# microsoft/UniSpeech

Measured on AMD Instinct MI355X. Metric: audio-seconds/sec pretraining, WavLM-Base 15s@16kHz, higher is better.
Workload: dtype bf16; 1 GPU; WavLM-Base (12L, d=768) pretrain fwd+bwd+grad-reduce+fused-Adam, bf16, batch=32x15s per GPU, masked-pred loss (BASELINE.json configs[1]); global_batch=32, frames_per_utt=749, parallelism=dp1, optimizer=fused Adam, fp32 master, clip 10

## Files before the change

### unispeech_amd/csrc/attn_fused.hip

```cpp
#include "attn_fused.hpp"

typedef float f32x2_t __attribute__((ext_vector_type(2)));
#if !defined(WAVLM_EXPERIMENTAL)
#undef FA_FWD_LAZY
#undef FA_FWD_THETA
#undef FA_DQ_PK
#endif
#ifndef FA_FWD_LAZY
#define FA_FWD_LAZY 0
#endif
#ifndef FA_FWD_THETA
#define FA_FWD_THETA 8.f
#endif
#ifndef FA_DQ_PK
#define FA_DQ_PK 1
#endif
#if !defined(WAVLM_EXPERIMENTAL)
#undef FA_FWD_MFMA_SUM
#endif
#ifndef FA_FWD_MFMA_SUM
#define FA_FWD_MFMA_SUM 0
#endif
#ifndef FA_FWD_BIAS_IN_C
#define FA_FWD_BIAS_IN_C 1
#endif
#ifndef FA_DQ_BIAS_IN_C
#define FA_DQ_BIAS_IN_C 0
#endif

template <bool DROP, bool STORE = false, bool BSTORE = false>
__global__ __launch_bounds__(256, 3) void attn_fwd_kernel(FaP p) {
  static_assert(!STORE || (FA_FWD_BIAS_IN_C && !FA_FWD_LAZY), "the probability store is written for the default forward");
  static_assert(!BSTORE || (DROP && !STORE && FA_FWD_BIAS_IN_C && !FA_FWD_LAZY), "the bit store is written for the default forward with dropout");
  extern __shared__ __attribute__((aligned(16))) unsigned char smem[];
  auto kbuf = [&](int st) { return smem + st * 16384; };
  auto vbuf = [&](int st) { return smem + st * 16384 + 8192; };
  float* tabs = reinterpret_cast<float*>(smem + 32768);
  float* kb = tabs + p.Ltab;
  unsigned* colw = reinterpret_cast<unsigned*>(kb + p.Tkb);
  const int T = p.T, H = p.H;
  int qblk, bh;
  fa_block_map(p.nqb, p.B * H, qblk, bh);
  const int b = bh / H, h = bh % H;
  const int lane = threadIdx.x & 63, wave = threadIdx.x >> 6;
  const int wave_u = __builtin_amdgcn_readfirstlane(wave);
  const int hi = lane >> 5, ql = lane & 31;
  const int i = qblk * FA_BQ + 32 * wave + ql;
  const int ic = i < T ? i : T - 1;
  const long D3 = 3L * H * FA_HD;
  const bf16_t* base = p.qkv + (long)b * T * D3 + h * FA_HD;
  const int L = 2 * T - 1;

  U4 qf[4];
#pragma unroll
  for (int kk = 0; kk < 4; ++kk) qf[kk].v = *reinterpret_cast<const uint4*>(base + (long)ic * D3 + 16 * kk + 8 * hi);
  for (int d = threadIdx.x; d < p.Ltab; d += 256) tabs[d] = (p.tab && d < L) ? p.tab[(long)h * L + d] : 0.f;
  for (int j = threadIdx.x; j < p.Tkb; j += 256)
    kb[j] = (j < T && !(p.kpm && p.kpm[(long)b * T + j])) ? 0.f : -INFINITY;
  if constexpr (DROP)
    for (int jp = threadIdx.x; jp < (p.Tkb >> 1); jp += 256) colw[jp] = fa_col_word(p.s1, (unsigned)jp);
  const float g2 = p.gate ? p.gate[(long)bh * T + ic] * FA_LOG2E : 0.f;
#if FA_FWD_BIAS_IN_C
  const float g2s = g2 / p.sc2;
#endif
  const unsigned roww = fa_row_word(p.s0, (unsigned)(bh * T + ic));
  const float* trow = tabs + (T - 1 - ic);

  f32x16_t o[2];
#pragma unroll
  for (int f = 0; f < 2; ++f)
#pragma unroll
    for (int r = 0; r < 16; ++r) o[f][r] = 0.f;
  float m = -INFINITY, l = 0.f;
#if FA_FWD_LAZY
  float mref = 0.f;
  bool seen = false;
#endif
  const int nkv = (T + FA_BKV - 1) / FA_BKV;
  const unsigned vtr = fa_tr_base(lane);
  unsigned* dbp = nullptr;
  if constexpr (BSTORE) dbp = p.dbits + ((long)bh * p.db_nkb + hi) * p.db_Tq + fa_bitrow(i);
  unsigned char* pst = nullptr;
  float* mtp = nullptr;
// ... 653 lines not shown
      }
    };
    auto dq_acc = [&](auto fc) __attribute__((always_inline)) {
      constexpr int f = decltype(fc)::value;
#pragma unroll
      for (int f2 = 0; f2 < 2; ++f2)
#pragma unroll
        for (int s2 = 0; s2 < 2; ++s2)
          dq[f2] = __builtin_amdgcn_mfma_f32_32x32x16_bf16(frag_tr(kbuf(cur), ktr, f2, f, s2), (f == 0 ? dsf0[s2] : dsf1[s2]).b, dq[f2], 0, 0, 0);
    };
#if FA_DQ_BOTH
    scores(F0{}); scores(F1{});
    if (edge) { elem_pass(F0{}, std::true_type{}); elem_pass(F1{}, std::true_type{}); }
    else { elem_pass(F0{}, std::false_type{}); elem_pass(F1{}, std::false_type{}); }
    dq_acc(F0{}); dq_acc(F1{});
#else
    scores(F0{});
    if (edge) elem_pass(F0{}, std::true_type{}); else elem_pass(F0{}, std::false_type{});
    dq_acc(F0{});
    scores(F1{});
    if (edge) elem_pass(F1{}, std::true_type{}); else elem_pass(F1{}, std::false_type{});
    dq_acc(F1{});
#endif
    if constexpr (EMIT) {
      auto spread = [&](unsigned a) __attribute__((always_inline)) {
        unsigned x = __builtin_bitreverse32(a) >> 16;
        x = (x | (x << 8)) & 0x00FF00FFu;
        x = (x | (x << 4)) & 0x0F0F0F0Fu;
        return x << (4 * hi);
      };
      unsigned w0 = spread(bacc0), w1 = spread(bacc1);
      asm volatile("s_nop 1\n\tv_permlane32_swap_b32 %0, %1\n\ts_nop 1" : "+v"(w0), "+v"(w1));
      pend_bits = w0 | w1;
      pend_bits_jt = jt;
      bacc0 = 0; bacc1 = 0;
    }
    if constexpr (TAB && !FA_DQ_DEFER) skew_sums(j0);
    fa_tile_sync<SP ? 5 : 0>();
    cur ^= 1;
  };
  if constexpr (SP) {
    for (int pi = 0; pi < (nkv >> 1); ++pi) {
      tile_body(2 * pi, pA0, pA1, mtA);
      tile_body(2 * pi + 1, pB0, pB1, mtB);
    }
    if (nkv & 1) tile_body(nkv - 1, pA0, pA1, mtA);
  } else {
    for (int jt = 0; jt < nkv; ++jt) tile_body(jt, pA0, pA1, mtA);
  }
  if constexpr (TAB && FA_DQ_DEFER) skew_sums((nkv - 1) * FA_BKV);
  if constexpr (TAB) flush_pending();
  if constexpr (EMIT)
    if (dbp && pend_bits_jt >= 0) dbp[(long)pend_bits_jt * 2 * p.db_Tq] = pend_bits;
  if (TAB && lane < 32) {
    const float v = lane < 16 ? dacc[4][0] : dacc[5][0];
    const int d = dlo0 + 64 * nkv + lane;
    if (d >= 0 && d < L) prow[d] = v;
  }
#if FA_DQ_PK
  dg = dg2[0] + dg2[1];
#endif
  dg = wl_sum_xor32(dg);
  if (p.dbias_part)
    fa_wave_colsum(dq, p.scale, reinterpret_cast<float*>(smem),
                   p.dbias_part + (((long)b * p.nqb + qblk) * 4 + wave_u) * D3 + h * FA_HD, lane, wave_u);
  if (valid_i) {
    bf16_t* dst = p.dqkv + ((long)b * T + i) * D3 + h * FA_HD;
#pragma unroll
    for (int f2 = 0; f2 < 2; ++f2)
#pragma unroll
      for (int q4 = 0; q4 < 4; ++q4) {
        uint2 w;
        w.x = pack_bf16(dq[f2][4 * q4] * p.scale, dq[f2][4 * q4 + 1] * p.scale);
        w.y = pack_bf16(dq[f2][4 * q4 + 2] * p.scale, dq[f2][4 * q4 + 3] * p.scale);
        *reinterpret_cast<uint2*>(dst + 32 * f2 + 8 * q4 + 4 * hi) = w;
      }
    if (hi == 0) {
      p.delta[(long)bh * T + i] = dl;
      if (p.dgate) p.dgate[(long)bh * T + i] = dg;
    }
  }
}

__global__ __launch_bounds__(1024) void fa_dtab_reduce_kernel(const float* __restrict__ part, float* __restrict__ out,
                                                              int B, int H, int nqt, int L, int Lp, int T, int nkv, int accumulate) {
  __shared__ float4 red[64][17];
  const int col = threadIdx.x & 15, slice = threadIdx.x >> 4;
  const int d = (blockIdx.x * 16 + col) * 4;
  const int h = blockIdx.y;
  const int nrow = nqt * 4, ntot = B * nrow, span = 64 * nkv + 32;
  float4 acc[4];
#pragma unroll
  for (int u = 0; u < 4; ++u) acc[u] = make_float4(0.f, 0.f, 0.f, 0.f);
  if (d < Lp) {
    for (int r0 = slice; r0 < ntot; r0 += 256) {
#pragma unroll
      for (int u = 0; u < 4; ++u) {
        const int r = r0 + 64 * u;
        if (r < ntot) {
          const int b = r / nrow, c = r - b * nrow;
          const int k0 = d - (T - 1 - 32 * c - 31);
          if (k0 > -4 && k0 < span) {
            const float4 v = *reinterpret_cast<const float4*>(part + (((long)b * H + h) * nrow + c) * Lp + d);
            acc[u].x += (k0 >= 0 && k0 < span) ? v.x : 0.f;
            acc[u].y += (k0 + 1 >= 0 && k0 + 1 < span) ? v.y : 0.f;
            acc[u].z += (k0 + 2 >= 0 && k0 + 2 < span) ? v.z : 0.f;
            acc[u].w += (k0 + 3 >= 0 && k0 + 3 < span) ? v.w : 0.f;
          }
        }
      }
    }
  }
  float4 t;
  t.x = (acc[0].x + acc[1].x) + (acc[2].x + acc[3].x); t.y = (acc[0].y + acc[1].y) + (acc[2].y + acc[3].y);
  t.z = (acc[0].z + acc[1].z) + (acc[2].z + acc[3].z); t.w = (acc[0].w + acc[1].w) + (acc[2].w + acc[3].w);
  red[slice][col] = t;
  __syncthreads();
  if (slice < 4) {
    float4 q = make_float4(0.f, 0.f, 0.f, 0.f);
#pragma unroll
    for (int k = 0; k < 16; ++k) { const float4 v = red[slice * 16 + k][col]; q.x += v.x; q.y += v.y; q.z += v.z; q.w += v.w; }
    red[slice * 16][col] = q;
  }
  __syncthreads();
  if (slice == 0 && d < L) {
    const float4 a0 = red[0][col], a1 = red[16][col], a2 = red[32][col], a3 = red[48][col];
    const float o[4] = {(a0.x + a1.x) + (a2.x + a3.x), (a0.y + a1.y) + (a2.y + a3.y), (a0.z + a1.z) + (a2.z + a3.z),
                        (a0.w + a1.w) + (a2.w + a3.w)};
#pragma unroll
    for (int k = 0; k < 4; ++k)
      if (d + k < L) out[(long)h * L + d + k] = accumulate ? out[(long)h * L + d + k] + o[k] : o[k];
  }
}

static FaP fa_params(int B, int H, int T, float scale, float p_drop, uint64_t seed) {
  FaP p;
  p.B = B; p.H = H; p.T = T; p.scale = scale;
  p.sc2 = scale * FA_LOG2E;
  double tt = (double)p_drop * 65536.0 + 0.5; if (tt > 65535.0) tt = 65535.0;
  p.th = p_drop > 0.f ? (unsigned)tt : 0u;
  if (p_drop > 0.f && p.th == 0u) p.th = 1u;
  p.sc = p.th ? (float)(1.0 / (1.0 - (double)p.th / 65536.0)) : 1.f;
  p.log2sc = log2f(p.sc); p.inv_sc = 1.f / p.sc;
  p.ths = (int)p.th - 32768;
  p.k2 = (unsigned)((p.ths - 1) & 0xffff) * 0x10001u;
  p.k3 = (unsigned)(p.ths & 0xffff) * 0x10001u;
  p.ps.P16 = nullptr; p.ps.mt = nullptr;
  p.dbits = nullptr; p.db_fwd = 0; p.db_nkb = ((T + FA_BKV - 1) / FA_BKV) * 2; p.db_Tq = ((T + FA_BQ - 1) / FA_BQ) * FA_BQ;
  p.ps.nq32 = ((T + FA_BQ - 1) / FA_BQ) * 4; p.ps.nkv = (T + FA_BKV - 1) / FA_BKV; p.ps.Tq = ((T + FA_BQ - 1) / FA_BQ) * FA_BQ;
  p.s0 = (unsigned)seed; p.s1 = (unsigned)(seed >> 32);
  const int nkv = (T + FA_BKV - 1) / FA_BKV;
  p.Tkb = nkv * FA_BKV;
  p.Ltab = (T + p.Tkb + 3) & ~3;
  p.qkv = nullptr; p.O = nullptr; p.lse = nullptr; p.gate = nullptr; p.tab = nullptr; p.kpm = nullptr;
  p.dO = nullptr; p.dqkv = nullptr; p.delta = nullptr; p.dgate = nullptr; p.dtab_part = nullptr; p.dbias_part = nullptr;
  return p;
}

extern "C" {

uint64_t wavlm_attn_fused_pstore_bytes(int32_t B, int32_t H, int32_t T) {
  if (B <= 0 || H <= 0 || T <= 0) return 0;
  if (T > FA_PSTORE_MAX_T) return 0;
  return ((fa_pstore_p_bytes(B, H, T) + 255) & ~(uint64_t)255) + fa_pstore_mt_bytes(B, H, T);
}

uint64_t wavlm_attn_fused_dbits_bytes(int32_t B, int32_t H, int32_t T) {
  if (B <= 0 || H <= 0 || T <= 0) return 0;
  return fa_dbits_bytes(B, H, T);
}

int wavlm_attn_fused_fwd(const void* qkv, void* O, float* lse, const float* gate, const float* tab, const uint8_t* kpm,
                         int32_t B, int32_t H, int32_t T, int32_t head_dim, float scale, float p_drop, uint64_t seed,
                         void* stream) {
  return wavlm_attn_fused_fwd_p(qkv, O, lse, gate, tab, kpm, nullptr, 0, B, H, T, head_dim, scale, p_drop, seed, stream);
}

static void fa_bind_pstore(FaP& p, void* pstore, int B, int H, int T) {
  p.ps.P16 = (unsigned char*)pstore;
  p.ps.mt = (float*)((unsigned char*)pstore + ((fa_pstore_p_bytes(B, H, T) + 255) & ~(uint64_t)255));
}

int wavlm_attn_fused_fwd_p(const void* qkv, void* O, float* lse, const float* gate, const float* tab, const uint8_t* kpm,
                           void* pstore, uint64_t pstore_bytes, int32_t B, int32_t H, int32_t T, int32_t head_dim, float scale,
                           float p_drop, uint64_t seed, void* stream) {
  if (!qkv || !O || !lse || B <= 0 || H <= 0 || T <= 0 || head_dim != FA_HD) return WL_EINVAL;
  if ((gate == nullptr) != (tab == nullptr)) return WL_EINVAL;
  const bool bitmode = pstore && pstore_bytes == fa_dbits_bytes(B, H, T);
  if (bitmode) { if ((uintptr_t)pstore & 255) return WL_EINVAL; }
  else if (pstore && (T > FA_PSTORE_MAX_T || pstore_bytes < wavlm_attn_fused_pstore_bytes(B, H, T) || ((uintptr_t)pstore & 15))) return WL_EINVAL;
  FaP p = fa_params(B, H, T, scale, p_drop, seed);
  p.qkv = (const bf16_t*)qkv; p.O = (bf16_t*)O; p.lse = lse; p.gate = gate; p.tab = tab; p.kpm = kpm;
  if (bitmode) { p.dbits = (unsigned*)pstore; p.db_fwd = 1; pstore = nullptr; }
  if (pstore) fa_bind_pstore(p, pstore, B, H, T);
  const size_t smem = 32768 + (size_t)(p.Ltab + p.Tkb + p.Tkb / 2) * sizeof(float);
  p.nqb = (T + FA_BQ - 1) / FA_BQ;
  const dim3 grid((unsigned)(p.nqb * B * H));
  WlProfScope prof(WL_PROF_ATTN_FWD, WL_BF16, 4.0 * B * H * (double)T * T * FA_HD,
                   (double)B * T * H * FA_HD * 2.0 * 4.0 + (double)B * H * T * 4.0, (hipStream_t)stream);
#define FA_FWD(DR, ST) do { if (fa_set_smem(attn_fwd_kernel<DR, ST>, smem) != WL_OK) return WL_ELAUNCH; \
    WL_LAUNCH((attn_fwd_kernel<DR, ST>), grid, dim3(256), smem, (hipStream_t)stream, p); } while (0)
  if (p.th && p.dbits) {
    if (fa_set_smem(attn_fwd_kernel<true, false, true>, smem) != WL_OK) return WL_ELAUNCH;
    WL_LAUNCH((attn_fwd_kernel<true, false, true>), grid, dim3(256), smem, (hipStream_t)stream, p);
  } else
  if (p.th) { if (pstore) FA_FWD(true, true); else FA_FWD(true, false); }
  else { if (pstore) FA_FWD(false, true); else FA_FWD(false, false); }
#undef FA_FWD
  return wl_check_launch();
}

uint64_t wavlm_attn_fused_bwd_workspace_bytes(int32_t B, int32_t H, int32_t T) {
  const uint64_t nqt = (uint64_t)((T + FA_BQ - 1) / FA_BQ);
  const uint64_t Lp = (2 * (uint64_t)T - 1 + 3) & ~(uint64_t)3;
  const uint64_t f = ((uint64_t)B * H * nqt * 4 * Lp + (uint64_t)B * H * T + (uint64_t)B * nqt * 4 * 3 * H * FA_HD) * sizeof(float);
// ... 22 lines not shown
}

int wl_attn_fused_bwd_ex(const void* qkv, const void* O, const void* dO, const float* lse, const float* gate,
                         const float* tab, const uint8_t* kpm, const void* pstore, uint64_t pstore_bytes, void* dqkv, float* dgate,
                         float* dtab, int dtab_accumulate,
                         void* dbias, int32_t dbias_dtype, int32_t dbias_accumulate, int32_t B, int32_t H, int32_t T,
                         int32_t head_dim, float scale, float p_drop, uint64_t seed, void* workspace, uint64_t ws_bytes,
                         void* stream) {
  if (!qkv || !O || !dO || !lse || !dqkv || !workspace || B <= 0 || H <= 0 || T <= 0 || head_dim != FA_HD)
    return WL_EINVAL;
  if ((gate == nullptr) != (tab == nullptr)) return WL_EINVAL;
  if (tab && (!dgate || !dtab)) return WL_EINVAL;
  if (ws_bytes < wavlm_attn_fused_bwd_workspace_bytes(B, H, T)) return WL_EINVAL;
  hipStream_t st = (hipStream_t)stream;
  FaP p = fa_params(B, H, T, scale, p_drop, seed);
  p.qkv = (const bf16_t*)qkv; p.O = (bf16_t*)const_cast<void*>(O); p.lse = const_cast<float*>(lse);
  p.gate = gate; p.tab = tab; p.kpm = kpm; p.dO = (const bf16_t*)dO; p.dqkv = (bf16_t*)dqkv; p.dgate = dgate;
  const unsigned* fwd_bits = nullptr;
  if (pstore && pstore_bytes == fa_dbits_bytes(B, H, T)) { fwd_bits = (const unsigned*)pstore; pstore = nullptr; }
  if (pstore) fa_bind_pstore(p, const_cast<void*>(pstore), B, H, T);
  const int nqt = (T + FA_BQ - 1) / FA_BQ;
  const int L = 2 * T - 1;
  p.dtab_part = (float*)workspace;
  const int Lp = (L + 3) & ~3;
  p.delta = p.dtab_part + (long)B * H * nqt * 4 * Lp;
  if (dbias) p.dbias_part = p.delta + (long)B * H * T;
  static const bool dbits_on = []() { const char* e = getenv("WAVLM_ATTN_DBITS"); return e && e[0] == '1'; }();
  static const bool dkv64_on = []() { const char* e = getenv("WAVLM_ATTN_DKV64"); return e && e[0] == '1'; }();
  bool use64 = dkv64_on && dbits_on && !pstore;
  if (use64) {
    FaP q = p; q.nqb = (T + FA_K64 - 1) / FA_K64;
    if (fa_dkv64_smem(q) > 160 * 1024) use64 = false;
  }
  if (fwd_bits && p.th) {
    p.dbits = const_cast<unsigned*>(fwd_bits); p.db_fwd = 1; use64 = false;
  } else
  if (dbits_on && !pstore && p.th) {
    const uint64_t fbytes = ((uint64_t)B * H * nqt * 4 * Lp + (uint64_t)B * H * T + (uint64_t)B * nqt * 4 * 3 * H * FA_HD) * sizeof(float);
    p.dbits = (unsigned*)((unsigned char*)workspace + ((fbytes + 255) & ~(uint64_t)255));
  }
  size_t smem1 = 32768 + (tab ? 4 * FA_SKEW_WAVE : 0) + (size_t)(p.Ltab + p.Tkb + p.Tkb / 2) * sizeof(float) + 256;
  if (smem1 < FA_CS_FLOATS * sizeof(float)) smem1 = FA_CS_FLOATS * sizeof(float);
  p.nqb = nqt;
  WlProfScope prof(WL_PROF_ATTN_BWD, WL_BF16, 10.0 * B * H * (double)T * T * FA_HD,
                   (double)B * T * H * FA_HD * 2.0 * 8.0 + (double)B * H * T * 8.0, st);
#define FA_DQ(DR, TB, SP_) do { if (fa_set_smem(attn_bwd_dq_kernel<DR, TB, SP_>, smem1) != WL_OK) return WL_ELAUNCH; \
    WL_LAUNCH((attn_bwd_dq_kernel<DR, TB, SP_>), dim3((unsigned)(nqt * B * H)), dim3(256), smem1, st, p); } while (0)
#define FA_DQB(TB) do { if (fa_set_smem(attn_bwd_dq_kernel<true, TB, false, true>, smem1) != WL_OK) return WL_ELAUNCH; \
    WL_LAUNCH((attn_bwd_dq_kernel<true, TB, false, true>), dim3((unsigned)(nqt * B * H)), dim3(256), smem1, st, p); } while (0)
  if (p.th && p.db_fwd) {
    if (tab) FA_DQB(true); else FA_DQB(false);
  } else
  if (pstore) {
    if (tab) FA_DQ(false, true, true); else FA_DQ(false, false, true);
  } else if (p.th && p.dbits) {
    if (tab) { if (fa_set_smem(attn_bwd_dq_kernel<true, true, false, false, true>, smem1) != WL_OK) return WL_ELAUNCH;
               WL_LAUNCH((attn_bwd_dq_kernel<true, true, false, false, true>), dim3((unsigned)(nqt * B * H)), dim3(256), smem1, st, p); }
    else { if (fa_set_smem(attn_bwd_dq_kernel<true, false, false, false, true>, smem1) != WL_OK) return WL_ELAUNCH;
           WL_LAUNCH((attn_bwd_dq_kernel<true, false, false, false, true>), dim3((unsigned)(nqt * B * H)), dim3(256), smem1, st, p); }
  } else if (p.th) {
    if (tab) FA_DQ(true, true, false); else FA_DQ(true, false, false);
  } else {
    if (tab) FA_DQ(false, true, false); else FA_DQ(false, false, false);
  }
#undef FA_DQ
#undef FA_DQB
  size_t smem2 = 32768 + (size_t)(p.Ltab + 64) * sizeof(float) + 2 * 4096;
  if (smem2 < FA_CS_FLOATS * sizeof(float)) smem2 = FA_CS_FLOATS * sizeof(float);
  if (use64) {
    p.nqb = (T + FA_K64 - 1) / FA_K64;
    const int rc = fa_launch_dkv64(p, (unsigned)(p.nqb * B * H), st);
    if (rc != WL_OK) return rc;
  } else {
    p.nqb = (T + FA_BK1 - 1) / FA_BK1;
    const dim3 grid2((unsigned)(p.nqb * B * H));
    const int rc = fa_launch_dkv(p, grid2.x, smem2, st);
    if (rc != WL_OK) return rc;
  }
  if (dbias) {
    const int rcb = wl_colsum_finish(p.dbias_part, B * nqt * 4, 3 * H * FA_HD, dbias, dbias_dtype, dbias_accumulate, st);
    if (rcb != WL_OK) return rcb;
    if (dbias_accumulate && !wl_fin_active()) wl_notify_grad(dbias, (uint64_t)3 * H * FA_HD * wl_esize(dbias_dtype), stream);
  }
  if (tab)
    WL_LAUNCH(fa_dtab_reduce_kernel, dim3((unsigned)((Lp / 4 + 15) / 16), (unsigned)H), dim3(1024), 0, st,
              (const float*)p.dtab_part, dtab, (int)B, (int)H, nqt, L, Lp, (int)T, (T + FA_BKV - 1) / FA_BKV, (int)dtab_accumulate);
  return wl_check_launch();
}
```

### unispeech_amd/csrc/common.hpp

```cpp
#pragma once
#include <hip/hip_runtime.h>
#include <stdint.h>
#include <stdio.h>
#include <mutex>

#define WL_MAX_DEVICES 64

#define WL_OK 0
#define WL_EINVAL (-1)
#define WL_ELAUNCH (-2)
#define WL_ENOMEM (-3)

enum { WL_F32 = 0, WL_BF16 = 1, WL_I16 = 2 };

typedef unsigned short bf16_t;

__device__ __forceinline__ float bf2f(bf16_t v) {
  return __uint_as_float(((unsigned)v) << 16);
}
__device__ __forceinline__ bf16_t f2bf(float f) {
  const __bf16 h = (__bf16)f;
  return __builtin_bit_cast(bf16_t, h);
}
__device__ __forceinline__ unsigned pack_bf16x2(float a, float b) {
// ... 89 lines not shown
}

__device__ __forceinline__ unsigned hash32(unsigned x) {
  x *= 0x9E3779B1u;
  x ^= x >> 15; x *= 0x85EBCA77u;
  x ^= x >> 13; x *= 0xC2B2AE3Du;
  x ^= x >> 16;
  return x;
}
__device__ __forceinline__ unsigned drop_mix(unsigned x) {
  x ^= x >> 16;
  unsigned r;
  asm("v_mul_u32_u24 %0, 0xb5297b, %1" : "=v"(r) : "v"(x));
  return r;
}
static inline unsigned drop_thresh16(float p) {
  if (p <= 0.f) return 0u;
  double t = (double)p * 65536.0 + 0.5;
  if (t > 65535.0) t = 65535.0;
  return t < 1.0 ? 1u : (unsigned)t;
}
static inline float drop_scale16(unsigned th16) { return th16 ? (float)(1.0 / (1.0 - (double)th16 / 65536.0)) : 1.f; }

struct Philox4 { unsigned x, y, z, w; };
__device__ __forceinline__ Philox4 philox4x32_10(unsigned long long seed, unsigned long long ctr) {
  unsigned k0 = (unsigned)seed, k1 = (unsigned)(seed >> 32);
  unsigned c0 = (unsigned)ctr, c1 = (unsigned)(ctr >> 32), c2 = 0x243F6A88u, c3 = 0x85A308D3u;
#pragma unroll
  for (int r = 0; r < 10; ++r) {
    const unsigned long long p0 = (unsigned long long)0xD2511F53u * c0;
    const unsigned long long p1 = (unsigned long long)0xCD9E8D57u * c2;
    const unsigned n0 = (unsigned)(p1 >> 32) ^ c1 ^ k0;
    const unsigned n1 = (unsigned)p1;
    const unsigned n2 = (unsigned)(p0 >> 32) ^ c3 ^ k1;
    const unsigned n3 = (unsigned)p0;
    c0 = n0; c1 = n1; c2 = n2; c3 = n3;
    k0 += 0x9E3779B9u; k1 += 0xBB67AE85u;
  }
  Philox4 o; o.x = c0; o.y = c1; o.z = c2; o.w = c3; return o;
}
__device__ __forceinline__ bool dropout_keep(unsigned long long seed, unsigned long long idx, unsigned thresh) {
  const Philox4 r = philox4x32_10(seed, idx >> 2);
  const unsigned sel = (unsigned)(idx & 3);
  const unsigned v = sel == 0 ? r.x : sel == 1 ? r.y : sel == 2 ? r.z : r.w;
  return v >= thresh;
}

static thread_local int wl_launch_failed = 0;
#define WL_LAUNCH(...)                                            \
  do {                                                            \
    (void)hipGetLastError();                                      \
    hipLaunchKernelGGL(__VA_ARGS__);                              \
    const hipError_t wl_e_ = hipGetLastError();                   \
    if (wl_e_ != hipSuccess) {                                    \
      wl_launch_failed = 1;                                       \
      fprintf(stderr, "[wavlm_hip] kernel launch failed: %s (%s:%d)\n", hipGetErrorString(wl_e_), __FILE__, __LINE__); \
    }                                                             \
  } while (0)
int wl_prof_begin(int cls, int dtype, double flops, double bytes, hipStream_t st);
void wl_prof_end(int i, hipStream_t st);
struct WlProfScope {
  int i; hipStream_t st;
  WlProfScope(int cls, int dtype, double flops, double bytes, hipStream_t s) : i(wl_prof_begin(cls, dtype, flops, bytes, s)), st(s) {}
  ~WlProfScope() { wl_prof_end(i, st); }
};

static inline int wl_check_launch() {
  const int e = wl_launch_failed;
  wl_launch_failed = 0;
  return e ? WL_ELAUNCH : WL_OK;
}

void wl_notify_grad(const void* base, uint64_t bytes, void* stream);
static inline uint64_t wl_esize(int dt) { return dt == WL_BF16 ? 2 : 4; }
int wl_attn_fused_bwd_ex(const void* qkv, const void* O, const void* dO, const float* lse, const float* gate,
                         const float* tab, const uint8_t* kpm, const void* pstore, uint64_t pstore_bytes, void* dqkv, float* dgate,
                         float* dtab, int dtab_accumulate,
                         void* dbias, int32_t dbias_dtype, int32_t dbias_accumulate, int32_t B, int32_t H, int32_t T,
                         int32_t head_dim, float scale, float p_drop, uint64_t seed, void* workspace, uint64_t ws_bytes,
                         void* stream);
int wl_colsum_finish(const float* part, int nblk, int n, void* out, int out_dtype, int accumulate, hipStream_t st);

struct WlFinSeg { const float* part; void* out; long stride, rep_stride; int nblk, n, out_dtype, accumulate, rep, blk0; };
#define WL_FIN_MAX 16
struct WlFinList { WlFinSeg s[WL_FIN_MAX]; int n, blocks; };
void wl_fin_defer(WlFinList* l);
bool wl_fin_active();
bool wl_fin_add(const float* part, int nblk, long stride, int n, void* out, int out_dtype, int accumulate, int rep = 1,
                long rep_stride = 0);
int wl_fin_flush(WlFinList& l, void* stream);
```

### unispeech_amd/csrc/gemm_bf16.hip

```cpp
#include <atomic>

#include "gemm_common.hpp"
#include "split_policy.hpp"

#include "tile_loaders.hpp"

template <bool TA, bool TB, int BM, int BN, int WM, int WN, bool VEC>
__global__ __launch_bounds__(WM * WN * 64) void gemm_bf16_kernel(GemmP p) {
  constexpr int FM = BM / WM / 32, FN = BN / WN / 32;
  constexpr int NT = WM * WN * 64;
  static_assert((WM * WN == 4 || WM * WN == 8) && FM >= 1 && FN >= 1, "4 or 8 waves");
  constexpr int A_BYTES = BM * 128, B_BYTES = BN * 128;
  extern __shared__ __attribute__((aligned(16))) unsigned char smem[];

  int tile;
  {
    const int nt = p.tiles_m * p.tiles_n, bid = blockIdx.x;
    const int q = nt >> 3, rem = nt & 7, xcd = bid & 7, idx = bid >> 3;
    tile = (xcd < rem ? xcd * (q + 1) : rem * (q + 1) + (xcd - rem) * q) + idx;
  }
  const int tn = tile % p.tiles_n, tm = tile / p.tiles_n;
  const int z = blockIdx.y, split = blockIdx.z;
  const int zo = z / p.batch_i, zi = z % p.batch_i;
  const int m0 = tm * BM, n0 = tn * BN;
// ... 83 lines not shown
      }
  } else {
    constexpr int WCOLS = BN / WN;
    constexpr int EP_LD = WCOLS + 4;
    constexpr int CH = WCOLS / 8;
    float* ep = reinterpret_cast<float*>(smem) + wave * (32 * EP_LD);
    const int zo2 = zo, zi2 = zi;
#pragma unroll
    for (int i = 0; i < FM; ++i) {
#pragma unroll
      for (int j = 0; j < FN; ++j)
#pragma unroll
        for (int r = 0; r < 16; ++r)
          ep[((r & 3) + 8 * (r >> 2) + 4 * (lane >> 5)) * EP_LD + j * 32 + (lane & 31)] = acc[i][j][r];
      __syncthreads();
#pragma unroll
      for (int q = 0; q < (32 * CH) / 64; ++q) {
        const int id = lane + 64 * q;
        const int rl = id / CH, ch = id % CH;
        const int mm = m0 + wm * (BM / WM) + i * 32 + rl;
        const int nn = n0 + wn * WCOLS + ch * 8;
        if (mm < p.M && nn < p.N) {
          const float4 lo = *reinterpret_cast<const float4*>(ep + rl * EP_LD + ch * 8);
          const float4 hi = *reinterpret_cast<const float4*>(ep + rl * EP_LD + ch * 8 + 4);
          float v[8] = {lo.x, lo.y, lo.z, lo.w, hi.x, hi.y, hi.z, hi.w};
          gemm_store8(p, zo2, zi2, z, split, mm, nn, v);
        }
      }
      __syncthreads();
    }
  }
}

__global__ __launch_bounds__(256) void gemm_splitk_reduce_kernel(GemmP p, int nbatch) {
  const long mn = (long)p.M * p.N;
  const long total = mn * nbatch;
  for (long i = (long)blockIdx.x * blockDim.x + threadIdx.x; i < total; i += (long)gridDim.x * blockDim.x) {
    const int z = (int)(i / mn);
    const long r = i - (long)z * mn;
    float s = 0.f;
    for (int k = 0; k < p.split_k; ++k) s += p.ws[((long)z * p.split_k + k) * mn + r];
    gemm_epi_final(p, z / p.batch_i, z % p.batch_i, (int)(r / p.N), (int)(r % p.N), s);
  }
}

__global__ __launch_bounds__(256) void gemm_splitk_reduce8_kernel(GemmP p, int nbatch) {
  const long mn = (long)p.M * p.N;
  const long total8 = (mn * nbatch) >> 3;
  const int S = p.split_k;
  GemmP q = p;
  q.split_k = 1;
  for (long i8 = (long)blockIdx.x * blockDim.x + threadIdx.x; i8 < total8; i8 += (long)gridDim.x * blockDim.x) {
    const long i = i8 << 3;
    const int z = (int)(i / mn);
    const long r = i - (long)z * mn;
    const float* src = p.ws + (long)z * S * mn + r;
    float v[8];
#pragma unroll
    for (int e = 0; e < 8; ++e) v[e] = 0.f;
    int k = 0;
    for (; k + 4 <= S; k += 4) {
      float4 a[4], b[4];
#pragma unroll
      for (int u = 0; u < 4; ++u) {
        a[u] = *reinterpret_cast<const float4*>(src + (long)(k + u) * mn);
        b[u] = *reinterpret_cast<const float4*>(src + (long)(k + u) * mn + 4);
      }
#pragma unroll
      for (int u = 0; u < 4; ++u) {
        v[0] += a[u].x; v[1] += a[u].y; v[2] += a[u].z; v[3] += a[u].w;
        v[4] += b[u].x; v[5] += b[u].y; v[6] += b[u].z; v[7] += b[u].w;
      }
    }
    for (; k < S; ++k) {
      const float4 a = *reinterpret_cast<const float4*>(src + (long)k * mn);
      const float4 b = *reinterpret_cast<const float4*>(src + (long)k * mn + 4);
      v[0] += a.x; v[1] += a.y; v[2] += a.z; v[3] += a.w; v[4] += b.x; v[5] += b.y; v[6] += b.z; v[7] += b.w;
    }
    const int m = (int)(r / p.N), n = (int)(r - (long)m * p.N);
    gemm_store8(q, z / p.batch_i, z % p.batch_i, z, 0, m, n, v);
  }
}

struct RedGrpP {
  float* ws[4]; void* C[4]; long ldc[4]; int M[4], N[4], c_dtype[4], accumulate[4]; float alpha[4];
  long base[5]; int n, S;
};
__global__ __launch_bounds__(256) void gemm_splitk_reduce8_grouped_kernel(RedGrpP p) {
  const long total8 = p.base[p.n];
  for (long i8 = (long)blockIdx.x * blockDim.x + threadIdx.x; i8 < total8; i8 += (long)gridDim.x * blockDim.x) {
    const int g = (i8 >= p.base[1]) + (i8 >= p.base[2]) + (i8 >= p.base[3]);
    const long i = (i8 - p.base[g]) << 3;
    const int N = p.N[g];
    const long mn = (long)p.M[g] * N;
    const float* src = p.ws[g] + i;
    float v[8];
#pragma unroll
    for (int e = 0; e < 8; ++e) v[e] = 0.f;
    for (int k = 0; k < p.S; ++k) {
      const float4 a = *reinterpret_cast<const float4*>(src + (long)k * mn);
      const float4 b = *reinterpret_cast<const float4*>(src + (long)k * mn + 4);
      v[0] += a.x; v[1] += a.y; v[2] += a.z; v[3] += a.w; v[4] += b.x; v[5] += b.y; v[6] += b.z; v[7] += b.w;
    }
    const long m = i / N, n = i - m * N;
    const long off = m * p.ldc[g] + n;
#pragma unroll
    for (int e = 0; e < 8; ++e) v[e] *= p.alpha[g];
    if (p.accumulate[g]) {
      float c[8];
      ld8_dt(p.C[g], off, p.c_dtype[g], c);
#pragma unroll
      for (int e = 0; e < 8; ++e) v[e] += c[e];
    }
    st8_dt(p.C[g], off, p.c_dtype[g], v);
  }
}

template <bool TA, bool TB, int BM, int BN, int WM, int WN>
static int launch_cfg(GemmP& p, int nbatch, bool vec, hipStream_t st) {
  p.tiles_m = (p.M + BM - 1) / BM;
  p.tiles_n = (p.N + BN - 1) / BN;
  dim3 grid((unsigned)(p.tiles_m * p.tiles_n), (unsigned)nbatch, (unsigned)p.split_k);
  constexpr size_t smem = 2 * (size_t)(BM + BN) * 128;
  constexpr int nt = WM * WN * 64;
  if (smem > 65536) {
    static bool done_v = false, done_s = false;
    bool& done = vec ? done_v : done_s;
    if (!done) {
      const void* fn = vec ? (const void*)gemm_bf16_kernel<TA, TB, BM, BN, WM, WN, true>
                           : (const void*)gemm_bf16_kernel<TA, TB, BM, BN, WM, WN, false>;
      if (hipFuncSetAttribute(fn, hipFuncAttributeMaxDynamicSharedMemorySize, (int)smem) != hipSuccess) return WL_ELAUNCH;
      done = true;
    }
  }
  if (vec) WL_LAUNCH((gemm_bf16_kernel<TA, TB, BM, BN, WM, WN, true>), grid, dim3(nt), smem, st, p);
  else WL_LAUNCH((gemm_bf16_kernel<TA, TB, BM, BN, WM, WN, false>), grid, dim3(nt), smem, st, p);
  return wl_check_launch();
}

static int g_gemm_variant = 0;
extern int g_pp_mode;
extern "C" void wavlm_gemm_set_variant(int v) { g_gemm_variant = v & 15; if (v >> 4) g_pp_mode = (v >> 4) - 1; }

template <bool TA, bool TB>
static int launch_t(GemmP& p, int nbatch, bool vec, hipStream_t st) {
  if (p.N <= 64) return launch_cfg<TA, TB, 128, 64, 2, 2>(p, nbatch, vec, st);
  if (g_gemm_variant == 2 ||
      (g_gemm_variant == 0 && p.M >= 2048 && (long)((p.M + 255) / 256) * ((p.N + 127) / 128) * nbatch * p.split_k >= 192))
    return launch_cfg<TA, TB, 256, 128, 4, 2>(p, nbatch, vec, st);
  return launch_cfg<TA, TB, 128, 128, 2, 2>(p, nbatch, vec, st);
}

static bool vec_epilogue_ok(const wavlm_gemm_desc* d, bool final_stage = false) {
  auto ok = [](const void* ptr, int64_t a, int64_t b, int64_t c) {
    return (((uintptr_t)ptr) & 15) == 0 && a % 8 == 0 && b % 8 == 0 && c % 8 == 0;
  };
  if (d->split_k > 1 && !final_stage) return (((uintptr_t)d->workspace) & 15) == 0 && d->N % 8 == 0;
  if (final_stage && d->N % 8) return false;
  if (!ok(d->C, d->ldc, d->sC_o, d->sC_i)) return false;
  if (d->bias && !ok(d->bias, 0, d->sBias_o, d->sBias_i)) return false;
  if (d->aux && !ok(d->aux, d->ld_aux, d->sAux_o, d->sAux_i)) return false;
  if (d->res && !ok(d->res, d->ld_res, d->sRes_o, d->sRes_i)) return false;
  return true;
}

int gemm_f32_launch(const wavlm_gemm_desc* d, hipStream_t st);
bool gemm_pp_ok(const wavlm_gemm_desc* d);
int gemm_pp_launch(GemmP& p, int nbatch, bool transA, bool transB, int ep, hipStream_t st);
bool gemm_pp3_ok(const wavlm_gemm_desc* d);
int gemm_pp3_launch(GemmP& p, int nbatch, bool transA, bool transB, int ep, hipStream_t st);
#if defined(WAVLM_EXPERIMENTAL)
#define GEMM_LAB 1
bool gemm_h2_ok(const wavlm_gemm_desc* d, int ec);
int gemm_h2_launch(GemmP& p, bool transB, int ep, hipStream_t st);
static int h2_mode() { static const int m = getenv("WAVLM_GEMM_H2") ? atoi(getenv("WAVLM_GEMM_H2")) : -1; return m; }
static bool h2_takes(const wavlm_gemm_desc* d, int ec) {
  const int m = h2_mode();
  if (m == 0 || !gemm_h2_ok(d, ec)) return false;
  if (m == 1) return true;
  return false;
}
#else
#define GEMM_LAB 0
#endif
int gemm_w4_launch(GemmP& p, int nbatch, bool transA, bool transB, int ep, hipStream_t st);
int gemm_w4_launch_grouped(GemmP& p, hipStream_t st);
static int w4_mode() { static const int m = getenv("WAVLM_GEMM_W4") ? atoi(getenv("WAVLM_GEMM_W4")) : 3; return m; }
static bool w4_takes(const wavlm_gemm_desc* d, bool grouped) {
  const int m = w4_mode();
  if (m == 1) return true;
  if (m == 2) return grouped || (d->transA && d->transB);
  if (m == 3) return grouped;
  return false;
}

static double tile_efficiency(const wavlm_gemm_desc* d, int nbatch, int BM, int BN) {
  const long tm = (d->M + BM - 1) / BM, tn = (d->N + BN - 1) / BN;
  const long tiles = tm * tn * nbatch * (d->split_k < 1 ? 1 : d->split_k);
// ... 219 lines not shown
      long blocks = ((total >> 3) + 255) / 256; if (blocks > 2048) blocks = 2048;
      WL_LAUNCH(gemm_splitk_reduce8_kernel, dim3((unsigned)blocks), dim3(256), 0, st, p, nbatch);
    } else {
      long blocks = (total + 255) / 256; if (blocks > 4096) blocks = 4096;
      WL_LAUNCH(gemm_splitk_reduce_kernel, dim3((unsigned)blocks), dim3(256), 0, st, p, nbatch);
    }
    rc = wl_check_launch();
  }
  if (rc == WL_OK && d->colsum) {
    if (csum_rows > 0) rc = wl_colsum_finish((const float*)d->workspace, csum_rows, d->N, d->colsum, d->colsum_dtype, d->colsum_accumulate, st);
    else rc = wavlm_colsum(d->C, d->M, d->N, d->ldc, d->c_dtype, nullptr, nullptr, d->colsum, d->colsum_dtype,
                           d->colsum_accumulate, d->workspace, d->ws_bytes, stream);
  }
  prof_end(pi, st);
  if (rc == WL_OK) gemm_notify(d, csum_rows > 0, stream);
  return rc;
}

int gemm_pp_launch_grouped(GemmP& p, hipStream_t st);
bool gemm_w4_fixup_ok(const GemmP& p);

extern "C" int wavlm_gemm_grouped(const wavlm_gemm_desc* d, int32_t n, void* stream) {
  if (!d || n <= 0) return WL_EINVAL;
  hipStream_t st = (hipStream_t)stream;
  bool ok = n >= 2 && n <= 4;
  for (int i = 0; ok && i < n; ++i) {
    const wavlm_gemm_desc* e = d + i;
    ok = e->A && e->B && e->C && e->workspace && e->dtype == WL_BF16 && e->transA && e->transB && e->KB <= 1 &&
         e->batch_o <= 1 && e->batch_i <= 1 && e->K == d->K && e->split_k == d->split_k && e->split_k >= 2 &&
         e->epi == 0 && !e->bias && !e->aux && !e->res && e->M > 0 && e->N > 0 && gemm_pp_ok(e) &&
         aligned16(e->A) && aligned16(e->B) && e->lda % 8 == 0 && e->ldb % 8 == 0 &&
         vec_epilogue_ok(e) && vec_epilogue_ok(e, true) && e->ws_bytes >= wavlm_gemm_workspace_bytes(e);
  }
  if (!ok || g_gemm_variant != 0) {
    for (int i = 0; i < n; ++i) {
      const int rc = wavlm_gemm(d + i, stream);
      if (rc != WL_OK) return rc;
    }
    return WL_OK;
  }
  GemmP p = make_gemm_params(d);
  p.ngrp = n;
  long tiles_all = 0;
  for (int i = 0; i < n; ++i) tiles_all += (long)((d[i].M + 255) / 256) * ((d[i].N + 255) / 256);
  const int G = wl_policy::grid_blocks();
  const bool sk_on = wl_policy::streamk();
  const int ksteps = (d->K + 63) / 64;
  GemmSk plan;
  const bool sk = sk_on && w4_takes(d, true) && tiles_all * (long)ksteps >= 8l * G && gemm_sk_plan(tiles_all, ksteps, G, plan) &&
                  d->split_k >= plan.s + 1;
  if (sk) p.split_k = plan.s + 1;
  else if (sk_on && !wl_policy::forced_split() && G / tiles_all >= 2 && d->split_k == G / tiles_all + 1)
    p.split_k = (int)(G / tiles_all);
  int vb = 0;
  double flops = 0.0;
  for (int i = 0; i < 4; ++i) {
    const wavlm_gemm_desc* e = d + (i < n ? i : n - 1);
    GemmGrp& g = p.grp[i];
    g.A = e->A; g.B = e->B; g.ws = (float*)e->workspace; g.lda = e->lda; g.ldb = e->ldb; g.M = e->M; g.N = e->N;
    g.tiles_m = (e->M + 255) / 256; g.tiles_n = (e->N + 255) / 256;
    g.C = e->C; g.ldc = e->ldc; g.c_dtype = e->c_dtype; g.accumulate = e->accumulate; g.alpha = e->alpha;
    g.vbase = i < n ? vb : 0x7fffffff;
    if (i < n) { vb += g.tiles_m * g.tiles_n * (sk ? 1 : p.split_k); flops += 2.0 * e->M * e->N * (double)e->K; }
  }
  p.vtotal = vb;
  if (sk) {
    p.sk_ks = ksteps; p.sk_wgs = G; p.sk_tiles = (int)tiles_all; p.sk_s = plan.s; p.sk_lm = plan.Lm;
    p.vtotal = G * plan.q;
    static const bool spread = [] { const char* e = getenv("WAVLM_SK_SPREAD"); return !(e && *e == '0'); }();
    p.sk_spread = spread && (plan.s * tiles_all) % 8 == 0 && plan.R % 8 == 0 && G % 8 == 0;
  }
  const int pi = prof_begin(d, st);
  if (pi >= 0) {
    g_prof.flops[pi] = flops;
    double by = 0.0;
    for (int i = 0; i < n; ++i) by += 2.0 * ((double)d[i].M * d[i].K + (double)d[i].N * d[i].K) + 2.0 * 2.0 * d[i].M * d[i].N;
    g_prof.bytes[pi] = by;
    int* sh = g_prof.shape[pi];
    sh[0] = -n; sh[1] = 0; sh[2] = d->K; sh[3] = 1; sh[4] = 3; sh[5] = 0; sh[6] = sk ? 0 : p.split_k; sh[7] = n;
  }
  const bool fixup = w4_takes(d, true) && gemm_w4_fixup_ok(p);
  p.fix_epoch = fixup ? 1u : 0u; p.fix_cnt = nullptr; p.fix_flag = nullptr;
  int rc = w4_takes(d, true) ? gemm_w4_launch_grouped(p, st) : gemm_pp_launch_grouped(p, st);
  if (rc == WL_OK && !fixup) {
    RedGrpP r;
    r.n = n; r.S = p.split_k; r.base[0] = 0;
    for (int i = 0; i < 4; ++i) {
      const wavlm_gemm_desc* e = d + (i < n ? i : n - 1);
      r.ws[i] = (float*)e->workspace; r.C[i] = e->C; r.ldc[i] = e->ldc; r.M[i] = e->M; r.N[i] = e->N;
      r.c_dtype[i] = e->c_dtype; r.accumulate[i] = e->accumulate; r.alpha[i] = e->alpha;
      r.base[i + 1] = i < n ? r.base[i] + (((long)e->M * e->N) >> 3) : 0x7fffffffffffffffL;
    }
    const long total8 = r.base[n];
    long blocks = (total8 + 255) / 256; if (blocks > 4096) blocks = 4096;
    WL_LAUNCH(gemm_splitk_reduce8_grouped_kernel, dim3((unsigned)blocks), dim3(256), 0, st, r);
    rc = wl_check_launch();
  }
  prof_end(pi, st);
  if (rc == WL_OK)
    for (int i = 0; i < n; ++i) gemm_notify(d + i, false, stream);
  return rc;
}
```

### unispeech_amd/csrc/gemm_common.hpp

```cpp
#pragma once
#include <stdlib.h>
#include "common.hpp"
#include "../../include/wavlm_hip.h"

struct GemmGrp { const void* A; const void* B; float* ws; long lda, ldb; int M, N, tiles_m, tiles_n, vbase;
                 void* C; long ldc; int c_dtype, accumulate; float alpha; };

struct GemmP {
  const void* A; const void* B; void* C;
  int M, N, K, KB;
  long lda, ldb, ldc, sA_kb, sB_kb;
  int batch_i;
  long sA_o, sA_i, sB_o, sB_i, sC_o, sC_i;
  float alpha; int epi; int c_dtype;
  const void* bias; int bias_dtype; long sBias_o, sBias_i;
  void* aux; int aux_dtype; long ld_aux, sAux_o, sAux_i;
  const void* res; int res_dtype; long ld_res, sRes_o, sRes_i;
  int accumulate;
  int split_k; float* ws;
  int tiles_m, tiles_n;
  int vtotal, nbatch, skew;
  int swz_r;
  int patch_m;
  int ngrp;
  unsigned fix_epoch; unsigned* fix_cnt; unsigned* fix_flag;
  int sk_ks, sk_wgs, sk_tiles, sk_s, sk_lm, sk_spread;
  const float4* gtab;
  float* colsum_part;
  GemmGrp grp[4];
};

#define GEMM_SK_SEG_COST 8
struct GemmSk { int s, R, q, Lm; };
static inline bool gemm_sk_plan(long T, long KS, int G, GemmSk& k) {
  if (T <= 0 || T >= G) return false;
  k.s = (int)(G / T); k.R = (int)(G - T * k.s);
  if (k.R == 0 || k.s < 1) return false;
  k.q = (int)((T + k.R - 1) / k.R);
  static const long c_env = [] { const char* e = getenv("WAVLM_SK_SEG_COST"); return e && *e ? atol(e) : 0l; }();
  const long c = c_env > 0 ? c_env : GEMM_SK_SEG_COST;
  const long L0 = (k.q * (KS + c) - c) / (1 + (long)k.s * k.q);
  long Lm = 0, best = 0;
  for (long L = L0; L <= L0 + 1; ++L) {
    if (L < 8 || KS - L * k.s < 1) continue;
    const long tail = k.q * (KS - L * k.s + c), cost = L + c > tail ? L + c : tail;
    if (Lm == 0 || cost < best) { Lm = L; best = cost; }
  }
  if (Lm == 0 || best * 100 > 97 * ((KS + k.s - 1) / k.s + c)) return false;
  k.Lm = (int)Lm;
  return true;
}

__host__ __device__ inline void gemm_tile_rc(int tile, int tiles_m, int tiles_n, int R, int& tm, int& tn) {
  if (R <= 1) { tm = tile / tiles_n; tn = tile - tm * tiles_n; return; }
  const int per = R * tiles_n;
  const int sr = tile / per;
  int rows = tiles_m - sr * R; if (rows > R) rows = R;
  const int w = tile - sr * per;
  tn = w / rows; tm = sr * R + (w - tn * rows);
}
static inline int gemm_pick_swizzle(int tile_m, int tile_n, int tiles_m, int tiles_n, long b_bytes) {
  static const int off = getenv("WAVLM_GEMM_SWIZZLE") && getenv("WAVLM_GEMM_SWIZZLE")[0] == '0';
  if (off || tiles_n <= 1 || tiles_m <= 1 || b_bytes < 6l * 1000 * 1000) return 0;
  long best = -1; int br = 0;
  for (int R = 1; R <= 32; R *= 2) {
    if (R > tiles_m) break;
    int cols = (32 + R - 1) / R; if (cols > tiles_n) cols = tiles_n;
    int rows = R; if (cols * R < 32) { rows = (32 + cols - 1) / cols; if (rows > tiles_m) rows = tiles_m; }
    const long cost = (long)tile_m * rows + (long)tile_n * cols;
    if (best < 0 || cost < best) { best = cost; br = R; }
  }
  return br <= 1 ? 0 : br;
}

static inline GemmP make_gemm_params(const wavlm_gemm_desc* d) {
  GemmP p;
  p.A = d->A; p.B = d->B; p.C = d->C;
  p.M = d->M; p.N = d->N; p.K = d->K; p.KB = d->KB < 1 ? 1 : d->KB;
  p.lda = d->lda; p.ldb = d->ldb; p.ldc = d->ldc; p.sA_kb = d->sA_kb; p.sB_kb = d->sB_kb;
  p.batch_i = d->batch_i < 1 ? 1 : d->batch_i;
  p.sA_o = d->sA_o; p.sA_i = d->sA_i; p.sB_o = d->sB_o; p.sB_i = d->sB_i; p.sC_o = d->sC_o; p.sC_i = d->sC_i;
  p.alpha = d->alpha; p.epi = d->epi; p.c_dtype = d->c_dtype;
  p.bias = d->bias; p.bias_dtype = d->bias_dtype; p.sBias_o = d->sBias_o; p.sBias_i = d->sBias_i;
  p.aux = d->aux; p.aux_dtype = d->aux_dtype; p.ld_aux = d->ld_aux; p.sAux_o = d->sAux_o; p.sAux_i = d->sAux_i;
  p.gtab = nullptr;
  p.colsum_part = nullptr;
  p.res = d->res; p.res_dtype = d->res_dtype; p.ld_res = d->ld_res; p.sRes_o = d->sRes_o; p.sRes_i = d->sRes_i;
  p.accumulate = d->accumulate;
  p.split_k = d->split_k < 1 ? 1 : d->split_k;
  p.ws = (float*)d->workspace;
  p.tiles_m = 0; p.tiles_n = 0; p.vtotal = 0; p.nbatch = 1; p.skew = 0; p.patch_m = 0; p.ngrp = 0;
  p.sk_ks = 0; p.sk_wgs = 0; p.sk_tiles = 0; p.sk_s = 0; p.sk_lm = 0; p.sk_spread = 0;
  p.swz_r = 0;
  p.fix_epoch = 0; p.fix_cnt = nullptr; p.fix_flag = nullptr;
  return p;
}

__device__ __forceinline__ void gemm_epi_final(const GemmP& p, int zo, int zi, int m, int n, float acc) {
  float v = p.alpha * acc;
  if (p.bias) v += ld_elem(p.bias, (long)zo * p.sBias_o + (long)zi * p.sBias_i + n, p.bias_dtype);
  if (p.epi == 1) {
    if (p.aux) st_elem(p.aux, (long)zo * p.sAux_o + (long)zi * p.sAux_i + (long)m * p.ld_aux + n, p.aux_dtype, v);
    v = gelu_f(v);
  } else if (p.epi == 2) {
    const float u = ld_elem(p.aux, (long)zo * p.sAux_o + (long)zi * p.sAux_i + (long)m * p.ld_aux + n, p.aux_dtype);
    v *= gelu_grad_f(u);
  } else if (p.epi == 3) {
    float gr;
    v = gelu_both_f(v, gr);
    if (p.aux) st_elem(p.aux, (long)zo * p.sAux_o + (long)zi * p.sAux_i + (long)m * p.ld_aux + n, p.aux_dtype, gr);
  } else if (p.epi == 4) {
    v *= ld_elem(p.aux, (long)zo * p.sAux_o + (long)zi * p.sAux_i + (long)m * p.ld_aux + n, p.aux_dtype);
  }
  if (p.res) v += ld_elem(p.res, (long)zo * p.sRes_o + (long)zi * p.sRes_i + (long)m * p.ld_res + n, p.res_dtype);
  const long ci = (long)zo * p.sC_o + (long)zi * p.sC_i + (long)m * p.ldc + n;
  if (p.accumulate) v += ld_elem(p.C, ci, p.c_dtype);
  st_elem(p.C, ci, p.c_dtype, v);
}

__device__ __forceinline__ void gemm_store(const GemmP& p, int z, int split, int m, int n, float acc) {
  if (p.split_k > 1) {
    p.ws[((long)z * p.split_k + split) * ((long)p.M * p.N) + (long)m * p.N + n] = acc;
  } else {
    gemm_epi_final(p, z / p.batch_i, z % p.batch_i, m, n, acc);
  }
}


__device__ __forceinline__ void ld8_dt(const void* p, long idx, int dt, float (&v)[8]) {
  if (dt == WL_F32) {
    const float4 a = *reinterpret_cast<const float4*>((const float*)p + idx);
    const float4 b = *reinterpret_cast<const float4*>((const float*)p + idx + 4);
    v[0] = a.x; v[1] = a.y; v[2] = a.z; v[3] = a.w; v[4] = b.x; v[5] = b.y; v[6] = b.z; v[7] = b.w;
  } else {
    const uint4 a = *reinterpret_cast<const uint4*>((const bf16_t*)p + idx);
    v[0] = __uint_as_float(a.x << 16); v[1] = __uint_as_float(a.x & 0xffff0000u);
    v[2] = __uint_as_float(a.y << 16); v[3] = __uint_as_float(a.y & 0xffff0000u);
    v[4] = __uint_as_float(a.z << 16); v[5] = __uint_as_float(a.z & 0xffff0000u);
    v[6] = __uint_as_float(a.w << 16); v[7] = __uint_as_float(a.w & 0xffff0000u);
  }
}
__device__ __forceinline__ void st8_dt(void* p, long idx, int dt, const float (&v)[8]) {
  if (dt == WL_F32) {
    *reinterpret_cast<float4*>((float*)p + idx) = make_float4(v[0], v[1], v[2], v[3]);
    *reinterpret_cast<float4*>((float*)p + idx + 4) = make_float4(v[4], v[5], v[6], v[7]);
  } else {
    uint4 o;
    o.x = pack_bf16x2(v[0], v[1]); o.y = pack_bf16x2(v[2], v[3]);
    o.z = pack_bf16x2(v[4], v[5]); o.w = pack_bf16x2(v[6], v[7]);
    *reinterpret_cast<uint4*>((bf16_t*)p + idx) = o;
  }
}

__device__ __forceinline__ void gemm_store8(const GemmP& p, int zo, int zi, int z, int split, int m, int n,
                                            float (&acc)[8]) {
  if (n + 8 > p.N) {
    for (int e = 0; e < 8 && n + e < p.N; ++e) gemm_store(p, z, split, m, n + e, acc[e]);
    return;
  }
  if (p.split_k > 1) {
    float* dst = p.ws + ((long)z * p.split_k + split) * ((long)p.M * p.N) + (long)m * p.N + n;
    *reinterpret_cast<float4*>(dst) = make_float4(acc[0], acc[1], acc[2], acc[3]);
    *reinterpret_cast<float4*>(dst + 4) = make_float4(acc[4], acc[5], acc[6], acc[7]);
    return;
  }
  float v[8];
#pragma unroll
  for (int e = 0; e < 8; ++e) v[e] = p.alpha * acc[e];
  if (p.bias) {
    float b[8];
    ld8_dt(p.bias, (long)zo * p.sBias_o + (long)zi * p.sBias_i + n, p.bias_dtype, b);
#pragma unroll
    for (int e = 0; e < 8; ++e) v[e] += b[e];
  }
  if (p.epi == 1) {
    if (p.aux) st8_dt(p.aux, (long)zo * p.sAux_o + (long)zi * p.sAux_i + (long)m * p.ld_aux + n, p.aux_dtype, v);
#pragma unroll
    for (int e = 0; e < 8; ++e) v[e] = gelu_f(v[e]);
  } else if (p.epi == 2) {
    float u[8];
    ld8_dt(p.aux, (long)zo * p.sAux_o + (long)zi * p.sAux_i + (long)m * p.ld_aux + n, p.aux_dtype, u);
#pragma unroll
    for (int e = 0; e < 8; ++e) v[e] *= gelu_grad_f(u[e]);
  } else if (p.epi == 3) {
    float gr[8];
#pragma unroll
    for (int e = 0; e < 8; ++e) v[e] = gelu_both_f(v[e], gr[e]);
    if (p.aux) st8_dt(p.aux, (long)zo * p.sAux_o + (long)zi * p.sAux_i + (long)m * p.ld_aux + n, p.aux_dtype, gr);
  } else if (p.epi == 4) {
    float u[8];
    ld8_dt(p.aux, (long)zo * p.sAux_o + (long)zi * p.sAux_i + (long)m * p.ld_aux + n, p.aux_dtype, u);
#pragma unroll
    for (int e = 0; e < 8; ++e) v[e] *= u[e];
  }
  if (p.res) {
    float r[8];
    ld8_dt(p.res, (long)zo * p.sRes_o + (long)zi * p.sRes_i + (long)m * p.ld_res + n, p.res_dtype, r);
#pragma unroll
    for (int e = 0; e < 8; ++e) v[e] += r[e];
  }
  const long ci = (long)zo * p.sC_o + (long)zi * p.sC_i + (long)m * p.ldc + n;
  if (p.accumulate) {
    float c[8];
    ld8_dt(p.C, ci, p.c_dtype, c);
#pragma unroll
    for (int e = 0; e < 8; ++e) v[e] += c[e];
  }
  st8_dt(p.C, ci, p.c_dtype, v);
}

#define GT4_N 2048
#define GT2_N (2 * GT4_N)
__device__ __forceinline__ float gelu_both_tab(const float4* tab4, float x, float& grad) {
  const float2* tab = reinterpret_cast<const float2*>(tab4);
  float u = fmaf(x, GT2_N / 16.0f, 8.0f * (GT2_N / 16.0f));
  u = __builtin_amdgcn_fmed3f(u, 0.f, (float)(GT2_N - 1));
  const float2 t = tab[(int)u];
  const float ph = fmaf(t.x, x, t.y);
  grad = fmaf(x, t.x, ph);
  return x * ph;
}
const float4* wl_gelu_tab4(hipStream_t st);
__device__ __forceinline__ void gelu_tab_stage(const float4* g, float4* lds) {
  for (int i = threadIdx.x; i < GT4_N; i += blockDim.x) lds[i] = g[i];
}

__device__ __forceinline__ void gemm_unpack8(const uint4& a, float (&u)[8]) {
  u[0] = __uint_as_float(a.x << 16); u[1] = __uint_as_float(a.x & 0xffff0000u);
  u[2] = __uint_as_float(a.y << 16); u[3] = __uint_as_float(a.y & 0xffff0000u);
  u[4] = __uint_as_float(a.z << 16); u[5] = __uint_as_float(a.z & 0xffff0000u);
  u[6] = __uint_as_float(a.w << 16); u[7] = __uint_as_float(a.w & 0xffff0000u);
}
template <int KIND>
__device__ __forceinline__ void gemm_store8_fast(const GemmP& p, int zo, int zi, int m, int n, const float (&acc)[8],
                                                 const float4* tab = nullptr, float* vout = nullptr, const uint4* aux_pre = nullptr,
// ... 94 lines not shown
```

### unispeech_amd/csrc/layer.hip

```cpp
#include <stdlib.h>
#include <string.h>

#include <atomic>

#include "common.hpp"
#include "split_policy.hpp"
#include "wavlm_hip.h"

static std::atomic<wavlm_grad_listener> g_listener{nullptr};
static std::atomic<void*> g_listener_user{nullptr};
void wl_notify_grad(const void* base, uint64_t bytes, void* stream) {
  const wavlm_grad_listener cb = g_listener.load(std::memory_order_acquire);
  if (cb && base && bytes) cb(base, bytes, stream, g_listener_user.load(std::memory_order_acquire));
}
extern "C" void wavlm_dp_set_listener(wavlm_grad_listener cb, void* user) {
  g_listener.store(nullptr, std::memory_order_release);
  g_listener_user.store(user, std::memory_order_release);
  g_listener.store(cb, std::memory_order_release);
}

namespace {

inline uint64_t rup256(uint64_t v) { return (v + 255) & ~(uint64_t)255; }

// ... 91 lines not shown
  gemm_base(g);
  g.c_dtype = pdt; g.M = w.N; g.N = w.K; g.K = (int32_t)n; g.transA = 1; g.transB = 1;
  g.lda = w.N; g.ldb = w.K; g.ldc = w.K; g.A = w.dy; g.B = w.x; g.C = w.dW; g.accumulate = 1; g.split_k = split;
}
inline long wg_tiles(const wavlm_wgrad_item& w) { return (long)((w.N + 255) / 256) * ((w.K + 255) / 256); }

#define RC(expr) do { const int rc_ = (expr); if (rc_ != WL_OK) return rc_; } while (0)

struct BwdWs {
  void *dsa, *df, *du, *dh, *dxa, *da, *dO, *dqkv;
  float* dgate;
  void *ln_ws, *ln_ws2, *cs_ws, *cs_ws2, *attn_ws, *gate_ws, *wg_ws;
  uint64_t ln_b, cs_b, attn_b, gate_b, wg_b, bytes;
};
BwdWs carve_bwd(const wavlm_layer_desc* d, void* base, uint64_t cap) {
  BwdWs w; memset(&w, 0, sizeof(w));
  Carver c(base ? base : (void*)256, base ? cap : (~(uint64_t)0 >> 1));
  const uint64_t n = (uint64_t)d->B * d->T, D = d->D, F = d->F;
  w.dsa = c.take(n * D * 2);
  w.df = d->p_drop > 0.f ? c.take(n * D * 2) : w.dsa;
  w.du = c.take(n * F * 2);
  w.dh = c.take(n * D * 2);
  w.dxa = c.take(n * D * 2);
  w.da = d->p_drop > 0.f ? c.take(n * D * 2) : w.dxa;
  w.dO = c.take(n * D * 2);
  w.dqkv = c.take(n * 3 * D * 2);
  if (d->tab) w.dgate = (float*)c.take((uint64_t)d->B * d->H * d->T * 4);
  w.ln_b = wavlm_layernorm_bwd_workspace_bytes(d->D); w.ln_ws = c.take(w.ln_b); w.ln_ws2 = c.take(w.ln_b);
  w.cs_b = lin_dx_colsum_ws((int64_t)n, d->F);
  if (w.cs_b < wavlm_colsum_workspace_bytes(d->D)) w.cs_b = wavlm_colsum_workspace_bytes(d->D);
  w.cs_ws = c.take(w.cs_b); w.cs_ws2 = c.take(w.cs_b);
  w.attn_b = wavlm_attn_fused_bwd_workspace_bytes(d->B, d->H, d->T); w.attn_ws = c.take(w.attn_b);
  w.gate_b = wavlm_gate_bwd_workspace_bytes(d->H, 64); w.gate_ws = c.take(w.gate_b);
  const wavlm_wgrad_item it[4] = {{nullptr, nullptr, nullptr, d->D, d->F}, {nullptr, nullptr, nullptr, d->F, d->D},
                                  {nullptr, nullptr, nullptr, d->D, d->D}, {nullptr, nullptr, nullptr, 3 * d->D, d->D}};
  w.wg_b = wavlm_linear_wgrads_workspace_bytes(it, 4, (int64_t)n); w.wg_ws = c.take(w.wg_b);
  w.bytes = c.off;
  if (base && !c.ok) w.bytes = ~(uint64_t)0;
  return w;
}

}

#if defined(WAVLM_EXPERIMENTAL)
extern "C" int wavlm_lab_build(void) { return 1; }
#endif

extern "C" {

static long grid_or(int32_t grid) { return grid > 0 ? grid : wl_policy::grid_blocks(); }
static int forced_or(int32_t forced) { return forced >= 0 ? forced : wl_policy::forced_split(); }
int32_t wavlm_grid_blocks(void) { return wl_policy::grid_blocks(); }
int32_t wavlm_wgrad_grouping(void) { return wl_policy::grouping() ? 1 : 0; }
int32_t wavlm_split_single(int32_t M, int32_t N, int64_t ktiles, int32_t grid) { return wl_policy::split_single(M, N, (long)ktiles, grid_or(grid)); }
int32_t wavlm_split_grouped(int64_t tiles, int64_t ktiles, int32_t grid, int32_t forced) {
  return wl_policy::split_grouped((long)tiles, (long)ktiles, grid_or(grid), forced_or(forced));
}
int32_t wavlm_slabs_grouped(int64_t tiles, int64_t ktiles, int32_t grid, int32_t forced, int32_t balanced) {
  return wl_policy::slabs_grouped((long)tiles, (long)ktiles, grid_or(grid), forced_or(forced), balanced >= 0 ? balanced != 0 : wl_policy::streamk());
}

uint64_t wavlm_linear_wgrads_workspace_bytes(const wavlm_wgrad_item* it, int32_t cnt, int64_t n) {
  if (!it || cnt <= 0 || n <= 0) return 0;
  uint64_t tot = 0;
  const long kt = (long)((n + 63) / 64), G = wl_policy::kFullGrid;
  const int forced = wl_policy::forced_split();
  const bool balanced = wl_policy::streamk() && forced == 0;
  for (int i = 0; i < cnt; ++i) {
    const long t = wg_tiles(it[i]);
    int s = wl_policy::split_single(it[i].N, it[i].K, kt, G);
    const int gs = wl_policy::slabs_grouped(t, kt, G, forced, false);
    if (gs > s) s = gs;
    if (balanced && t < G && G / t + 1 > s) s = (int)(G / t) + 1;
    tot += rup256((uint64_t)s * it[i].N * it[i].K * 4);
  }
  return tot;
}

int wavlm_linear_wgrads(const wavlm_wgrad_item* it, int32_t cnt, int64_t n, int32_t pdt, void* ws, uint64_t wsb, void* stream) {
  if (!it || cnt <= 0 || n <= 0 || (pdt != WL_BF16 && pdt != WL_F32)) return WL_EINVAL;
  for (int i = 0; i < cnt; ++i)
    if (!it[i].dy || !it[i].x || !it[i].dW || it[i].N <= 0 || it[i].K <= 0) return WL_EINVAL;
  const long kt = (long)((n + 63) / 64);
  int i = 0;
  while (i < cnt) {
    int j = i; long tiles = 0;
    while (wl_policy::grouping() && j < cnt && j - i < 4) {
      const long t = wg_tiles(it[j]);
      if (j > i && wavlm_split_grouped(tiles + t, kt, 0, -1) < 2) break;
      tiles += t; ++j;
    }
    if (j == i) j = i + 1;
    const int m = j - i;
    Carver c(ws, wsb);
    if (m >= 2) {
      const int split = wavlm_slabs_grouped(tiles, kt, 0, -1, -1);
      wavlm_gemm_desc g[4];
      for (int k = 0; k < m; ++k) {
        wg_desc(g[k], it[i + k], n, pdt, split);
        g[k].ws_bytes = wavlm_gemm_workspace_bytes(&g[k]);
        g[k].workspace = c.take(g[k].ws_bytes);
      }
      if (!c.ok) return WL_EINVAL;
      const int rc = wavlm_gemm_grouped(g, m, stream);
      if (rc != WL_OK) return rc;
    } else {
      wavlm_gemm_desc g;
      wg_desc(g, it[i], n, pdt, wavlm_split_single(it[i].N, it[i].K, kt, 0));
      if (g.split_k > 1) { g.ws_bytes = wavlm_gemm_workspace_bytes(&g); g.workspace = c.take(g.ws_bytes); if (!c.ok) return WL_EINVAL; }
      const int rc = wavlm_gemm(&g, stream);
      if (rc != WL_OK) return rc;
    }
    i = j;
  }
  return WL_OK;
}

uint64_t wavlm_layer_saved_bytes(const wavlm_layer_desc* d) { return desc_ok(d) ? carve_saved(d, nullptr).bytes : 0; }

uint64_t wavlm_layer_fwd_workspace_bytes(const wavlm_layer_desc* d) {
  if (!desc_ok(d)) return 0;
  return rup256((uint64_t)d->B * d->T * d->D * 2) + (d->saved ? 0 : carve_saved(d, nullptr).bytes);
}

uint64_t wavlm_layer_bwd_workspace_bytes(const wavlm_layer_desc* d) { return desc_ok(d) ? carve_bwd(d, nullptr, 0).bytes : 0; }

int wavlm_encoder_layer_fwd(const wavlm_layer_desc* d, void* stream) {
  if (!desc_ok(d) || !d->x || !d->y || !d->workspace) return WL_EINVAL;
  if (d->pre_ln && !d->r_out) return WL_EINVAL;
  if (d->ws_bytes < wavlm_layer_fwd_workspace_bytes(d)) return WL_EINVAL;
  const int64_t n = (int64_t)d->B * d->T;
  const int D = d->D, F = d->F, pdt = d->param_dtype;
  Carver wc(d->workspace, d->ws_bytes);
  void* tmp = wc.take((uint64_t)n * D * 2);
  void* sbase = d->saved;
  if (sbase) { if (d->saved_bytes < carve_saved(d, nullptr).bytes) return WL_EINVAL; }
  else sbase = wc.take(carve_saved(d, nullptr).bytes);
  if (!wc.ok) return WL_EINVAL;
  const Saved s = carve_saved(d, sbase);

  const void* ain = d->x;
  if (d->pre_ln) {
    RC(wavlm_layernorm_fwd(d->x, d->r_in, s.h1, d->r_in ? s.s1 : nullptr, s.mean1, s.rstd1, d->ln1_g, d->ln1_b, n, D, d->eps1,
                           WL_BF16, pdt, 0, d->r_in ? d->p_drop : 0.f, d->seed_r1, 0.f, 0, stream));
    ain = s.h1;
  }
  const float* gate = nullptr;
  if (d->Wgate) {
    RC(wavlm_gate_fwd(ain, d->Wgate, d->bgate, d->grep_a, s.gate, s.ga, s.gb, d->B, d->T, d->H, 64, WL_BF16, pdt, stream));
    gate = s.gate;
  } else if (d->tab) {
    return WL_EINVAL;
  }
  RC(lin_fwd(ain, d->Wqkv, d->bqkv, s.qkv, n, 3 * D, D, pdt, 0, nullptr, stream));
  RC(wavlm_attn_fused_fwd_p(s.qkv, s.O, s.lse, gate, d->tab, d->kpm, d->saved ? s.pstore : nullptr, s.pstore_b, d->B, d->H, d->T, 64,
                            d->scale, d->p_attn, d->seed_attn, stream));
  RC(lin_fwd(s.O, d->Wo, d->bo, tmp, n, D, D, pdt, 0, nullptr, stream));
  if (!d->pre_ln) {
    RC(wavlm_layernorm_fwd(d->x, tmp, s.x1, s.s1, s.mean1, s.rstd1, d->ln1_g, d->ln1_b, n, D, d->eps1, WL_BF16, pdt, 0,
                           d->p_drop, d->seed_r1, 0.f, 0, stream));
    RC(lin_fwd(s.x1, d->W1, d->b1, s.hact, n, F, D, pdt, 3, s.u, stream));
    RC(lin_fwd(s.hact, d->W2, d->b2, tmp, n, D, F, pdt, 0, nullptr, stream));
    RC(wavlm_layernorm_fwd(s.x1, tmp, d->y, s.s2, s.mean2, s.rstd2, d->ln2_g, d->ln2_b, n, D, d->eps2, WL_BF16, pdt, 0,
                           d->p_drop, d->seed_r2, 0.f, 0, stream));
  } else {
    const void* s1 = d->r_in ? s.s1 : d->x;
    RC(wavlm_layernorm_fwd(s1, tmp, s.x1, d->y, s.mean2, s.rstd2, d->ln2_g, d->ln2_b, n, D, d->eps2, WL_BF16, pdt, 0,
                           d->p_drop, d->seed_r2, 0.f, 0, stream));
    RC(lin_fwd(s.x1, d->W1, d->b1, s.hact, n, F, D, pdt, 3, s.u, stream));
    RC(lin_fwd(s.hact, d->W2, d->b2, d->r_out, n, D, F, pdt, 0, nullptr, stream));
  }
  return WL_OK;
}

int wavlm_encoder_layer_bwd(const wavlm_layer_desc* d, void* stream) {
  if (!desc_ok(d) || !d->x || !d->dy || !d->dx || !d->saved || !d->workspace) return WL_EINVAL;
  if (!d->dWqkv || !d->dbqkv || !d->dWo || !d->dbo || !d->dW1 || !d->db1 || !d->dW2 || (!d->db2 && !d->pre_ln)) return WL_EINVAL;
// ... 71 lines not shown
```

### unispeech_amd/csrc/posconv.hip

```cpp
#include "common.hpp"
#include "../../include/wavlm_hip.h"

#define PC_BLOCKS 512

template <typename TA, typename TB>
__global__ void pc_rowdot_partial_kernel(const TA* __restrict__ a, const TB* __restrict__ b, long rows, int K,
                                         float* __restrict__ part) {
  const int k = threadIdx.x;
  if (k >= K) return;
  float s0 = 0.f, s1 = 0.f, s2 = 0.f, s3 = 0.f;
  const long G = gridDim.x;
  long r = blockIdx.x;
  for (; r + 3 * G < rows; r += 4 * G) {
    s0 = fmaf(Elem<TA>::ld(a + r * K + k), Elem<TB>::ld(b + r * K + k), s0);
    s1 = fmaf(Elem<TA>::ld(a + (r + G) * K + k), Elem<TB>::ld(b + (r + G) * K + k), s1);
    s2 = fmaf(Elem<TA>::ld(a + (r + 2 * G) * K + k), Elem<TB>::ld(b + (r + 2 * G) * K + k), s2);
    s3 = fmaf(Elem<TA>::ld(a + (r + 3 * G) * K + k), Elem<TB>::ld(b + (r + 3 * G) * K + k), s3);
  }
  for (; r < rows; r += G) s0 = fmaf(Elem<TA>::ld(a + r * K + k), Elem<TB>::ld(b + r * K + k), s0);
  part[(long)blockIdx.x * K + k] = (s0 + s1) + (s2 + s3);
}

__global__ __launch_bounds__(1024) void pc_finish_kernel(const float* __restrict__ part, int nblk, int K, float* __restrict__ tot, int do_sqrt) {
  __shared__ double red[64][17];
  const int col = threadIdx.x & 15, slice = threadIdx.x >> 4;
  const int k = blockIdx.x * 16 + col;
  double s = 0.0;
  if (k < K)
    for (int b = slice; b < nblk; b += 64) s += part[(long)b * K + k];
  red[slice][col] = s;
  __syncthreads();
  if (slice == 0 && k < K) {
    s = 0.0;
    for (int j = 0; j < 64; ++j) s += red[j][col];
    tot[k] = do_sqrt ? (float)sqrt(s) : (float)s;
  }
}

template <typename TP, typename TO>
__global__ __launch_bounds__(256) void pc_weight_kernel(const TP* __restrict__ v, const TP* __restrict__ g,
    const float* __restrict__ norm, TO* __restrict__ Wf, TO* __restrict__ Wb, int D, int Cg, int K, int layout) {
  const long total = (long)D * Cg * K;
  const long KC = (long)K * Cg;
  auto off = [&](int grp, int n, int tap, int c) -> long {
    if (layout == 0) return ((long)grp * Cg + n) * KC + (long)tap * Cg + c;
    const int J = K >> 4;
    return (long)grp * Cg * KC + (((((long)(c >> 3) * 4 + ((tap & 15) >> 2)) * J + (tap >> 4)) * 4 + (tap & 3)) * Cg + n) * 8 + (c & 7);
  };
  for (long i = (long)blockIdx.x * blockDim.x + threadIdx.x; i < total; i += (long)gridDim.x * blockDim.x) {
    const int k = (int)(i % K);
    const long r = i / K;
    const int ci = (int)(r % Cg), co = (int)(r / Cg);
    const int grp = co / Cg, col = co % Cg;
    const float nrm = norm[k];
    const float w = Elem<TP>::ld(g + k) * Elem<TP>::ld(v + i) / nrm;
    Elem<TO>::st(Wf + off(grp, col, k, ci), w);
    Elem<TO>::st(Wb + off(grp, ci, K - 1 - k, col), w);
  }
}

__global__ __launch_bounds__(256) void pc_unpack_dw_kernel(const float* __restrict__ dWf, float* __restrict__ dw, int D,
                                                           int Cg, int K, int nsplit) {
  extern __shared__ float pc_tile[];
  const int co = blockIdx.x;
  const long n = (long)K * Cg, total = (long)D * n;
  const float* src = dWf + (long)co * n;
  for (int i = threadIdx.x; i < (int)n; i += 256) {
    float a = src[i];
    for (int sidx = 1; sidx < nsplit; ++sidx) a += src[sidx * total + i];
    const int k = i / Cg, ci = i - k * Cg;
    pc_tile[k * (Cg + 1) + ci] = a;
  }
  __syncthreads();
  float* dst = dw + (long)co * n;
  for (int i = threadIdx.x; i < (int)n; i += 256) {
    const int ci = i / K, k = i - ci * K;
    dst[i] = pc_tile[k * (Cg + 1) + ci];
  }
}
template <typename TP>
__global__ __launch_bounds__(256) void pc_weight_bwd_kernel(const float* __restrict__ dw, const TP* __restrict__ v,
    const TP* __restrict__ g, const float* __restrict__ norm, const float* __restrict__ Stot,
    TP* __restrict__ dv, TP* __restrict__ dg, int D, int Cg, int K) {
  const long total = (long)D * Cg * K;
  for (long i = (long)blockIdx.x * blockDim.x + threadIdx.x; i < total; i += (long)gridDim.x * blockDim.x) {
    const int k = (int)(i % K);
    const float S = Stot[k];
    const float n = norm[k];
    const float gk = Elem<TP>::ld(g + k);
    Elem<TP>::st(dv + i, gk / n * (dw[i] - Elem<TP>::ld(v + i) * S / (n * n)));
    if (i < K) Elem<TP>::st(dg + k, S / n);
  }
}

template <typename T>
__global__ __launch_bounds__(256) void pc_group_major_kernel(const T* __restrict__ x, const T* __restrict__ aux,
    T* __restrict__ out, T* __restrict__ nat, int B, int Tn, int D, int G, int left_pad, int Tp, int aux_is_grad) {
  const int Cg = D / G, c8n = Cg >> 3;
  const long total = (long)B * G * Tp * c8n;
  for (unsigned i = blockIdx.x * blockDim.x + threadIdx.x; i < (unsigned)total; i += gridDim.x * blockDim.x) {
    const int c8 = (int)(i % (unsigned)c8n);
    unsigned r = i / (unsigned)c8n;
    const int tp = (int)(r % (unsigned)Tp); r /= (unsigned)Tp;
    const int g = (int)(r % (unsigned)G);
    const int b = (int)(r / (unsigned)G);
    const int t = tp - left_pad;
    unsigned short o[8];
#pragma unroll
    for (int e = 0; e < 8; ++e) o[e] = 0;
    float v[8];
#pragma unroll
    for (int e = 0; e < 8; ++e) v[e] = 0.f;
    if (t >= 0 && t < Tn) {
      const long src = ((long)b * Tn + t) * D + g * Cg + c8 * 8;
#pragma unroll
      for (int e = 0; e < 8; ++e) v[e] = Elem<T>::ld(x + src + e);
      if (aux) {
#pragma unroll
        for (int e = 0; e < 8; ++e) {
          const float a = Elem<T>::ld(aux + src + e);
          v[e] *= aux_is_grad ? a : gelu_grad_f(a);
        }
      }
      if (nat) {
#pragma unroll
        for (int e = 0; e < 8; ++e) Elem<T>::st(nat + src + e, v[e]);
      }
    }
    const long dst = (((long)b * G + g) * Tp + tp) * Cg + c8 * 8;
#pragma unroll
    for (int e = 0; e < 8; ++e) Elem<T>::st(out + dst + e, v[e]);
  }
}

extern "C" {

uint64_t wavlm_posconv_weight_workspace_bytes(int32_t D, int32_t Cg, int32_t K) {
  return ((uint64_t)(PC_BLOCKS + 1) * K + (uint64_t)D * Cg * K) * sizeof(float);
}

int wavlm_posconv_weight_fwd(const void* v, const void* g, int32_t param_dtype, void* Wf, void* Wb, int32_t out_dtype,
                             float* norm, int32_t D, int32_t Cg, int32_t K, int32_t layout, void* workspace,
                             uint64_t ws_bytes, void* stream) {
  if (!v || !g || !Wf || !Wb || !norm || !workspace || D <= 0 || Cg <= 0 || K <= 0 || K > 1024 || D % Cg) return WL_EINVAL;
  if (layout != 0 && (layout != 1 || (K & 15) || (Cg & 7))) return WL_EINVAL;
  if (ws_bytes < wavlm_posconv_weight_workspace_bytes(D, Cg, K)) return WL_EINVAL;
  hipStream_t st = (hipStream_t)stream;
  float* part = (float*)workspace;
  const long rows = (long)D * Cg;
  const unsigned th = (unsigned)((K + 63) / 64 * 64);
  const long total = rows * K;
  long grid = (total + 255) / 256; if (grid > 4096) grid = 4096;
  if (param_dtype == WL_F32) {
    WL_LAUNCH((pc_rowdot_partial_kernel<float, float>), dim3(PC_BLOCKS), dim3(th), 0, st, (const float*)v,
                       (const float*)v, rows, (int)K, part);
    WL_LAUNCH(pc_finish_kernel, dim3((unsigned)((K + 15) / 16)), dim3(1024), 0, st, part, PC_BLOCKS, (int)K, norm, 1);
    if (out_dtype == WL_F32)
      WL_LAUNCH((pc_weight_kernel<float, float>), dim3((unsigned)grid), dim3(256), 0, st, (const float*)v,
                         (const float*)g, norm, (float*)Wf, (float*)Wb, (int)D, (int)Cg, (int)K, (int)layout);
    else
      WL_LAUNCH((pc_weight_kernel<float, bf16_t>), dim3((unsigned)grid), dim3(256), 0, st, (const float*)v,
                         (const float*)g, norm, (bf16_t*)Wf, (bf16_t*)Wb, (int)D, (int)Cg, (int)K, (int)layout);
  } else if (param_dtype == WL_BF16 && out_dtype == WL_BF16) {
    WL_LAUNCH((pc_rowdot_partial_kernel<bf16_t, bf16_t>), dim3(PC_BLOCKS), dim3(th), 0, st, (const bf16_t*)v,
                       (const bf16_t*)v, rows, (int)K, part);
    WL_LAUNCH(pc_finish_kernel, dim3((unsigned)((K + 15) / 16)), dim3(1024), 0, st, part, PC_BLOCKS, (int)K, norm, 1);
    WL_LAUNCH((pc_weight_kernel<bf16_t, bf16_t>), dim3((unsigned)grid), dim3(256), 0, st, (const bf16_t*)v,
                       (const bf16_t*)g, norm, (bf16_t*)Wf, (bf16_t*)Wb, (int)D, (int)Cg, (int)K, (int)layout);
  } else return WL_EINVAL;
  return wl_check_launch();
}

int wavlm_posconv_weight_bwd(const float* dWf, const void* v, const void* g, const float* norm, int32_t param_dtype,
                             void* dv, void* dg, int32_t D, int32_t Cg, int32_t K, int32_t nsplit, void* workspace,
                             uint64_t ws_bytes, void* stream) {
  if (!dWf || !v || !g || !norm || !dv || !dg || !workspace || D <= 0 || Cg <= 0 || K <= 0 || K > 1024 || D % Cg || nsplit < 1)
    return WL_EINVAL;
  if ((size_t)K * (Cg + 1) * sizeof(float) > 65536) return WL_EINVAL;
  if (ws_bytes < wavlm_posconv_weight_workspace_bytes(D, Cg, K)) return WL_EINVAL;
  hipStream_t st = (hipStream_t)stream;
  float* part = (float*)workspace;
  float* Stot = part + (long)PC_BLOCKS * K;
  float* dw = Stot + K;
  const long rows = (long)D * Cg;
  const long total = rows * K;
  long grid = (total + 255) / 256; if (grid > 4096) grid = 4096;
  const unsigned th = (unsigned)((K + 63) / 64 * 64);
  WL_LAUNCH(pc_unpack_dw_kernel, dim3((unsigned)D), dim3(256), (size_t)K * (Cg + 1) * sizeof(float), st, dWf, dw, (int)D, (int)Cg, (int)K, (int)nsplit);
  if (param_dtype == WL_F32) {
    WL_LAUNCH((pc_rowdot_partial_kernel<float, float>), dim3(PC_BLOCKS), dim3(th), 0, st, (const float*)dw,
                       (const float*)v, rows, (int)K, part);
    WL_LAUNCH(pc_finish_kernel, dim3((unsigned)((K + 15) / 16)), dim3(1024), 0, st, part, PC_BLOCKS, (int)K, Stot, 0);
    WL_LAUNCH((pc_weight_bwd_kernel<float>), dim3((unsigned)grid), dim3(256), 0, st, (const float*)dw,
                       (const float*)v, (const float*)g, norm, Stot, (float*)dv, (float*)dg, (int)D, (int)Cg, (int)K);
  } else if (param_dtype == WL_BF16) {
    WL_LAUNCH((pc_rowdot_partial_kernel<float, bf16_t>), dim3(PC_BLOCKS), dim3(th), 0, st, (const float*)dw,
                       (const bf16_t*)v, rows, (int)K, part);
    WL_LAUNCH(pc_finish_kernel, dim3((unsigned)((K + 15) / 16)), dim3(1024), 0, st, part, PC_BLOCKS, (int)K, Stot, 0);
    WL_LAUNCH((pc_weight_bwd_kernel<bf16_t>), dim3((unsigned)grid), dim3(256), 0, st, (const float*)dw,
                       (const bf16_t*)v, (const bf16_t*)g, norm, Stot, (bf16_t*)dv, (bf16_t*)dg, (int)D, (int)Cg, (int)K);
  } else return WL_EINVAL;
  return wl_check_launch();
}

int wavlm_posconv_group_major(const void* x, const void* aux, void* out, void* nat_out, int32_t B, int32_t T, int32_t D,
                              int32_t G, int32_t left_pad, int32_t Tp, int32_t dtype, int32_t aux_is_grad, void* stream) {
  if (!x || !out || B <= 0 || T <= 0 || D <= 0 || G <= 0 || D % G || ((D / G) & 7) || left_pad < 0 || Tp < left_pad + T)
    return WL_EINVAL;
  hipStream_t st = (hipStream_t)stream;
  const long total = (long)B * G * Tp * ((D / G) >> 3);
  if (total >= (1L << 31) - 8192L * 256) return WL_EINVAL;
  long grid = (total + 255) / 256; if (grid > 8192) grid = 8192;
  if (dtype == WL_F32)
    WL_LAUNCH((pc_group_major_kernel<float>), dim3((unsigned)grid), dim3(256), 0, st, (const float*)x,
                       (const float*)aux, (float*)out, (float*)nat_out, (int)B, (int)T, (int)D, (int)G, (int)left_pad, (int)Tp, (int)aux_is_grad);
  else if (dtype == WL_BF16)
    WL_LAUNCH((pc_group_major_kernel<bf16_t>), dim3((unsigned)grid), dim3(256), 0, st, (const bf16_t*)x,
                       (const bf16_t*)aux, (bf16_t*)out, (bf16_t*)nat_out, (int)B, (int)T, (int)D, (int)G, (int)left_pad,
                       (int)Tp, (int)aux_is_grad);
  else return WL_EINVAL;
  return wl_check_launch();
}

}
```

### unispeech_amd/csrc/rowops.hip

```cpp
#include "common.hpp"
#include <stdlib.h>
#include "../../include/wavlm_hip.h"

__device__ __forceinline__ void load8(const float* p, float (&v)[8]) {
  const float4 a = *reinterpret_cast<const float4*>(p);
  const float4 b = *reinterpret_cast<const float4*>(p + 4);
  v[0] = a.x; v[1] = a.y; v[2] = a.z; v[3] = a.w; v[4] = b.x; v[5] = b.y; v[6] = b.z; v[7] = b.w;
}
__device__ __forceinline__ void load8(const bf16_t* p, float (&v)[8]) {
  const uint4 a = *reinterpret_cast<const uint4*>(p);
  v[0] = __uint_as_float(a.x << 16); v[1] = __uint_as_float(a.x & 0xffff0000u);
  v[2] = __uint_as_float(a.y << 16); v[3] = __uint_as_float(a.y & 0xffff0000u);
  v[4] = __uint_as_float(a.z << 16); v[5] = __uint_as_float(a.z & 0xffff0000u);
  v[6] = __uint_as_float(a.w << 16); v[7] = __uint_as_float(a.w & 0xffff0000u);
}
__device__ __forceinline__ void store8(float* p, const float (&v)[8]) {
  *reinterpret_cast<float4*>(p) = make_float4(v[0], v[1], v[2], v[3]);
  *reinterpret_cast<float4*>(p + 4) = make_float4(v[4], v[5], v[6], v[7]);
}
__device__ __forceinline__ void store8(bf16_t* p, const float (&v)[8]) {
  uint4 o;
  o.x = pack_bf16x2(v[0], v[1]); o.y = pack_bf16x2(v[2], v[3]);
  o.z = pack_bf16x2(v[4], v[5]); o.w = pack_bf16x2(v[6], v[7]);
  *reinterpret_cast<uint4*>(p) = o;
}
__device__ __forceinline__ unsigned keep8(unsigned long long seed, unsigned long long idx, unsigned thresh) {
  const Philox4 a = philox4x32_10(seed, idx >> 2), b = philox4x32_10(seed, (idx >> 2) + 1);
  return (a.x >= thresh ? 1u : 0u) | (a.y >= thresh ? 2u : 0u) | (a.z >= thresh ? 4u : 0u) | (a.w >= thresh ? 8u : 0u) |
         (b.x >= thresh ? 16u : 0u) | (b.y >= thresh ? 32u : 0u) | (b.z >= thresh ? 64u : 0u) | (b.w >= thresh ? 128u : 0u);
}
static inline unsigned drop_thresh(float p) {
  if (p <= 0.f) return 0u;
  double t = (double)p * 4294967296.0;
  if (t > 4294967295.0) t = 4294967295.0;
  return (unsigned)t;
}

#define LN_MAXC 4

template <int NC>
__device__ __forceinline__ void ln_drop_cols(unsigned long long seed_in, unsigned long long seed_out, int lane, int nch,
                                             unsigned (&cw)[NC][4]) {
  const unsigned k = (unsigned)seed_in * 0x2545F491u + (unsigned)seed_out + 0x7F4A7C15u;
#pragma unroll
  for (int c = 0; c < NC; ++c) {
    const int ch = lane + 64 * c;
#pragma unroll
    for (int j = 0; j < 4; ++j) cw[c][j] = ch < nch ? hash32(k ^ (unsigned)(ch * 4 + j)) : 0u;
  }
}
__device__ __forceinline__ unsigned ln_drop_row(unsigned long long seed, long row) {
  return hash32((unsigned)(seed >> 32) + (unsigned)row * 0x27D4EB2Fu + ((unsigned)seed ^ 0x165667B1u));
}
__device__ __forceinline__ void ln_drop_apply(float (&v)[8], unsigned rw, const unsigned (&cw)[4], unsigned th, float sc) {
#pragma unroll
  for (int j = 0; j < 4; ++j) {
    const unsigned w = drop_mix(rw + cw[j]);
    v[2 * j] = (w & 0xffffu) >= th ? v[2 * j] * sc : 0.f;
    v[2 * j + 1] = (w >> 16) >= th ? v[2 * j + 1] * sc : 0.f;
  }
}

template <typename T, typename TP, int NC>
__global__ __launch_bounds__(256) void layernorm_fwd_kernel(const T* __restrict__ x, const T* __restrict__ r, T* __restrict__ y,
    T* __restrict__ s, float* __restrict__ mean_o, float* __restrict__ rstd_o, const TP* __restrict__ gamma,
    const TP* __restrict__ beta, long rows, int D, float eps, int act, unsigned th_in, float sc_in,
    unsigned long long seed_in, unsigned th_out, float sc_out, unsigned long long seed_out) {
  const int lane = threadIdx.x & 63, wave = threadIdx.x >> 6;
  const int nch = D >> 3;
  unsigned cw[NC][4];
  if (th_in | th_out) ln_drop_cols<NC>(seed_in, seed_out, lane, nch, cw);
  for (long row = (long)blockIdx.x * 4 + wave; row < rows; row += (long)gridDim.x * 4) {
    float v[NC][8];
    float sum = 0.f;
    const unsigned rw_in = th_in ? ln_drop_row(seed_in, row) : 0u, rw_out = th_out ? ln_drop_row(seed_out, row) : 0u;
#pragma unroll
    for (int c = 0; c < NC; ++c) {
      const int ch = lane + 64 * c;
      if (ch < nch) {
        const long off = row * D + ch * 8;
        load8(x + off, v[c]);
        if (r) {
          float rv[8];
// ... 392 lines not shown
#pragma unroll
    for (int c = 0; c < NC; ++c) {
      const long off = row * D + (lane + 64 * c) * VEC;
      const long ooff = orow * D + (lane + 64 * c) * VEC;
      float o[VEC];
#pragma unroll
      for (int e = 0; e < VEC; ++e) o[e] = grad_scale * rstd * (h[c][e] - s1 - xh[c][e] * s2);
      if constexpr (HA) {
        float t[VEC];
#pragma unroll
        for (int e = 0; e < VEC; ++e) t[e] = o[e] + addv[c][e];
        stv<VEC>(dx + ooff, t);
        if (dr_incl_add) {
#pragma unroll
          for (int e = 0; e < VEC; ++e) o[e] = t[e];
        }
      } else stv<VEC>(dx + ooff, o);
      if constexpr (HD || CS) {
        if (th_in) lnf_drop_apply<VEC>(o, rw_in, cw[c], th_in, sc_in);
        if constexpr (HD) stv<VEC>(dr + off, o);
        if constexpr (CS) {
#pragma unroll
          for (int e = 0; e < VEC; ++e) ac[c][e] += o[e];
        }
      }
    }
  }
  float* pg = part + (long)blockIdx.x * NA * D;
#pragma unroll
  for (int c = 0; c < NC; ++c) {
    __syncthreads();
#pragma unroll
    for (int e = 0; e < VEC; ++e) {
      red[wave][0][lane * VEC + e] = ag[c][e]; red[wave][1][lane * VEC + e] = ab[c][e];
      if constexpr (CS) red[wave][2][lane * VEC + e] = ac[c][e];
    }
    __syncthreads();
    for (int i = threadIdx.x; i < 64 * VEC; i += 256) {
      const int col = c * 64 * VEC + i;
      pg[col] = red[0][0][i] + red[1][0][i] + red[2][0][i] + red[3][0][i];
      pg[D + col] = red[0][1][i] + red[1][1][i] + red[2][1][i] + red[3][1][i];
      if constexpr (CS) pg[2 * D + col] = red[0][2][i] + red[1][2][i] + red[2][2][i] + red[3][2][i];
    }
  }
}

__global__ __launch_bounds__(1024) void colsum_finish_kernel(const float* __restrict__ part, int nblk, long stride, int n,
                                                              void* out, int out_dtype, int accumulate, long part_y, void* out_y,
                                                              void* out_z) {
  __shared__ float red[64][17];
  const int col = threadIdx.x & 15, slice = threadIdx.x >> 4;
  const int c = blockIdx.x * 16 + col;
  if (blockIdx.y) { part += part_y * blockIdx.y; out = blockIdx.y == 1 ? out_y : out_z; }
  float s = 0.f;
  if (c < n) {
    float s0 = 0.f, s1 = 0.f, s2 = 0.f, s3 = 0.f;
    int b = slice;
    for (; b + 192 < nblk; b += 256) {
      s0 += part[(long)b * stride + c];
      s1 += part[(long)(b + 64) * stride + c];
      s2 += part[(long)(b + 128) * stride + c];
      s3 += part[(long)(b + 192) * stride + c];
    }
    for (; b < nblk; b += 64) s0 += part[(long)b * stride + c];
    s = (s0 + s1) + (s2 + s3);
  }
  red[slice][col] = s;
  __syncthreads();
  if (slice < 4) {
    float t = 0.f;
#pragma unroll
    for (int k = 0; k < 16; ++k) t += red[slice * 16 + k][col];
    red[slice * 16][col] = t;
  }
  __syncthreads();
  if (slice == 0 && c < n) {
    s = (red[0][col] + red[16][col]) + (red[32][col] + red[48][col]);
    if (accumulate) s += ld_elem(out, c, out_dtype);
    st_elem(out, c, out_dtype, s);
  }
}

__global__ __launch_bounds__(1024) void colsum_finish_multi_kernel(WlFinList L) {
  __shared__ float red[64][17];
  int si = 0;
#pragma unroll 1
  for (int k = 1; k < L.n; ++k) if ((int)blockIdx.x >= L.s[k].blk0) si = k;
  const WlFinSeg& g = L.s[si];
  const float* __restrict__ part = g.part;
  const long stride = g.stride;
  const int nblk = g.nblk, n = g.n;
  const int col = threadIdx.x & 15, slice = threadIdx.x >> 4;
  const int c = ((int)blockIdx.x - g.blk0) * 16 + col;
  float s = 0.f;
  if (c < n) {
    float s0 = 0.f, s1 = 0.f, s2 = 0.f, s3 = 0.f;
    int b = slice;
    for (; b + 192 < nblk; b += 256) {
      s0 += part[(long)b * stride + c];
      s1 += part[(long)(b + 64) * stride + c];
      s2 += part[(long)(b + 128) * stride + c];
      s3 += part[(long)(b + 192) * stride + c];
    }
    for (; b < nblk; b += 64) s0 += part[(long)b * stride + c];
    s = (s0 + s1) + (s2 + s3);
  }
  red[slice][col] = s;
  __syncthreads();
  if (slice < 4) {
    float t = 0.f;
#pragma unroll
    for (int k = 0; k < 16; ++k) t += red[slice * 16 + k][col];
    red[slice * 16][col] = t;
  }
  __syncthreads();
  if (slice == 0 && c < n) {
    s = (red[0][col] + red[16][col]) + (red[32][col] + red[48][col]);
    for (int r = 0; r < g.rep; ++r) {
      const long idx = (long)r * g.rep_stride + c;
      st_elem(g.out, idx, g.out_dtype, g.accumulate ? s + ld_elem(g.out, idx, g.out_dtype) : s);
    }
  }
}

static thread_local WlFinList* g_fin_list = nullptr;
void wl_fin_defer(WlFinList* l) { g_fin_list = l; if (l) { l->n = 0; l->blocks = 0; } }
bool wl_fin_active() { return g_fin_list != nullptr; }
bool wl_fin_add(const float* part, int nblk, long stride, int n, void* out, int out_dtype, int accumulate, int rep, long rep_stride) {
  WlFinList* l = g_fin_list;
  if (!l || l->n >= WL_FIN_MAX || n <= 0) return false;
  WlFinSeg& g = l->s[l->n++];
  g.part = part; g.out = out; g.stride = stride; g.rep_stride = rep_stride; g.nblk = nblk; g.n = n; g.out_dtype = out_dtype;
  g.accumulate = accumulate; g.rep = rep < 1 ? 1 : rep; g.blk0 = l->blocks;
  l->blocks += (n + 15) / 16;
  return true;
}
int wl_fin_flush(WlFinList& l, void* stream) {
  if (l.n == 0) return WL_OK;
  WL_LAUNCH(colsum_finish_multi_kernel, dim3((unsigned)l.blocks), dim3(1024), 0, (hipStream_t)stream, l);
  const int rc = wl_check_launch();
  if (rc == WL_OK)
    for (int k = 0; k < l.n; ++k) {
      const WlFinSeg& g = l.s[k];
      if (g.accumulate) wl_notify_grad(g.out, (uint64_t)((long)(g.rep - 1) * g.rep_stride + g.n) * wl_esize(g.out_dtype), stream);
    }
  l.n = 0; l.blocks = 0;
  return rc;
}

#define CS_MAXC 8
template <typename T>
__global__ __launch_bounds__(256) void colsum_partial_kernel(const T* __restrict__ x, long rows, int N, long ld,
    const unsigned char* __restrict__ inc, const unsigned char* __restrict__ exc, float* __restrict__ part) {
  __shared__ float red[4][512];
  const int lane = threadIdx.x & 63, wave = threadIdx.x >> 6;
  const int nch = N >> 3;
  float acc[CS_MAXC][8];
#pragma unroll
  for (int c = 0; c < CS_MAXC; ++c)
#pragma unroll
    for (int e = 0; e < 8; ++e) acc[c][e] = 0.f;
  for (long row = (long)blockIdx.x * 4 + wave; row < rows; row += (long)gridDim.x * 4) {
    if (inc && !inc[row]) continue;
    if (exc && exc[row]) continue;
#pragma unroll
    for (int c = 0; c < CS_MAXC; ++c) {
      const int ch = lane + 64 * c;
      if (ch < nch) {
        float v[8];
        load8(x + row * ld + ch * 8, v);
#pragma unroll
        for (int e = 0; e < 8; ++e) acc[c][e] += v[e];
      }
    }
  }
  float* pg = part + (long)blockIdx.x * N;
#pragma unroll
  for (int c = 0; c < CS_MAXC; ++c) {
    __syncthreads();
#pragma unroll
    for (int e = 0; e < 8; ++e) red[wave][lane * 8 + e] = acc[c][e];
    __syncthreads();
    for (int i = threadIdx.x; i < 512; i += 256) {
      const int ch = (i >> 3) + 64 * c;
      if (ch < nch) pg[ch * 8 + (i & 7)] = red[0][i] + red[1][i] + red[2][i] + red[3][i];
    }
  }
}

template <typename T, typename TP>
__global__ __launch_bounds__(256) void select_rows_kernel(const T* __restrict__ x, T* __restrict__ y,
    const unsigned char* __restrict__ sel, const TP* __restrict__ emb, const unsigned char* __restrict__ zero,
    long rows, int D) {
  const int nch = D >> 3;
  const long total = rows * nch;
  for (long i = (long)blockIdx.x * blockDim.x + threadIdx.x; i < total; i += (long)gridDim.x * blockDim.x) {
    const long row = i / nch; const int ch = (int)(i - row * nch);
    float v[8];
    if (zero && zero[row]) {
#pragma unroll
      for (int e = 0; e < 8; ++e) v[e] = 0.f;
    } else if (sel && sel[row]) {
      if (emb) load8(emb + ch * 8, v);
      else {
#pragma unroll
        for (int e = 0; e < 8; ++e) v[e] = 0.f;
      }
    } else {
      load8(x + row * D + ch * 8, v);
    }
    store8(y + row * D + ch * 8, v);
  }
}

template <typename T>
__global__ __launch_bounds__(256) void gather_rows_kernel(const T* __restrict__ src, const int* __restrict__ idx,
                                                           T* __restrict__ dst, long n_out, int D) {
  const int nch = D >> 3;
  const long total = n_out * nch;
  for (long i = (long)blockIdx.x * blockDim.x + threadIdx.x; i < total; i += (long)gridDim.x * blockDim.x) {
    const long row = i / nch; const int ch = (int)(i - row * nch);
    const int srow = idx[row];
    float v[8];
    if (srow >= 0) load8(src + (long)srow * D + ch * 8, v);
    else {
#pragma unroll
      for (int e = 0; e < 8; ++e) v[e] = 0.f;
    }
    store8(dst + row * D + ch * 8, v);
// ... 54 lines not shown
                                                           const unsigned char* __restrict__ sel, T* __restrict__ y, long n8,
                                                           int d8, unsigned th, float sc, unsigned long long seed) {
  const bool small = n8 <= 0xffffffffL, drop = th != 0u || sc != 1.f;
  for (long i = (long)blockIdx.x * blockDim.x + threadIdx.x; i < n8; i += (long)gridDim.x * blockDim.x) {
    float v[8];
    load8((sel[chunk_row(i, d8, small)] ? q : x) + i * 8, v);
    if (drop) {
      const unsigned k = keep8(seed, (unsigned long long)i * 8, th);
#pragma unroll
      for (int e = 0; e < 8; ++e) v[e] = ((k >> e) & 1u) ? v[e] * sc : 0.f;
    }
    store8(y + i * 8, v);
  }
}
template <typename T>
__global__ __launch_bounds__(256) void replace_mix_bwd_kernel(const T* __restrict__ g, const unsigned char* __restrict__ sel,
                                                               T* __restrict__ dx, T* __restrict__ dq, long n8, int d8,
                                                               unsigned th, float sc, unsigned long long seed) {
  const bool small = n8 <= 0xffffffffL, drop = th != 0u || sc != 1.f;
  for (long i = (long)blockIdx.x * blockDim.x + threadIdx.x; i < n8; i += (long)gridDim.x * blockDim.x) {
    float v[8], z[8];
    load8(g + i * 8, v);
    if (drop) {
      const unsigned k = keep8(seed, (unsigned long long)i * 8, th);
#pragma unroll
      for (int e = 0; e < 8; ++e) v[e] = ((k >> e) & 1u) ? v[e] * sc : 0.f;
    }
    const bool s = sel[chunk_row(i, d8, small)] != 0;
#pragma unroll
    for (int e = 0; e < 8; ++e) {
      z[e] = s ? 0.f : v[e];
      v[e] = s ? v[e] : 0.f;
    }
    store8(dx + i * 8, z);
    store8(dq + i * 8, v);
  }
}

template <typename T>
__global__ __launch_bounds__(256) void sumsq_partial_kernel(const T* __restrict__ x, long n, double* part) {
  __shared__ double red[4];
  float a[8];
#pragma unroll
  for (int e = 0; e < 8; ++e) a[e] = 0.f;
  const long nv = n >> 3;
  for (long i = (long)blockIdx.x * blockDim.x + threadIdx.x; i < nv; i += (long)gridDim.x * blockDim.x) {
    float v[8];
    load8(x + i * 8, v);
#pragma unroll
    for (int e = 0; e < 8; ++e) a[e] = fmaf(v[e], v[e], a[e]);
  }
  double s = ((double)a[0] + a[1]) + ((double)a[2] + a[3]) + ((double)a[4] + a[5]) + ((double)a[6] + a[7]);
  if (blockIdx.x == 0 && threadIdx.x < (n & 7)) {
    const float v = Elem<T>::ld(x + nv * 8 + threadIdx.x);
    s += (double)v * v;
  }
  s = wave_sum_d(s);
  if ((threadIdx.x & 63) == 0) red[threadIdx.x >> 6] = s;
  __syncthreads();
  if (threadIdx.x == 0) part[blockIdx.x] = red[0] + red[1] + red[2] + red[3];
}
__global__ __launch_bounds__(64) void sum_finish_d_kernel(const double* part, int n, float* out, float scale) {
  double s = 0.0;
  for (int i = threadIdx.x; i < n; i += 64) s += part[i];
  s = wave_sum_d(s);
  if (threadIdx.x == 0) out[0] = (float)(s * scale);
}

static inline unsigned grid_for(long work_items, int per_block, unsigned cap) {
  long g = (work_items + per_block - 1) / per_block;
  if (g < 1) g = 1;
  if (g > cap) g = cap;
  return (unsigned)g;
}

#ifndef LN_BWD_BLOCKS
#define LN_BWD_BLOCKS 512
#endif
#ifndef LN_FWD_DROP_BLOCKS
#define LN_FWD_DROP_BLOCKS 1024
#endif
#define CS_BLOCKS 512

__global__ __launch_bounds__(256) void conv_weights_relayout_kernel(wavlm_conv_relayout_desc d) {
  const int l = blockIdx.y;
  const int Cout = d.Cout[l], Cin = d.Cin[l], k = d.k[l], st = d.s[l];
  const long n = (long)Cout * Cin * k;
  for (long e = (long)blockIdx.x * 256 + threadIdx.x; e < n; e += (long)gridDim.x * 256) {
    const int kk = (int)(e % k);
    const long t = e / k;
    const int ci = (int)(t % Cin), co = (int)(t / Cin);
    const float v = ld_elem(d.W[l], e, d.dtype);
    st_elem(d.Wf[l], (long)co * (k * Cin) + (long)kk * Cin + ci, d.dtype, v);
    if (d.Wb[l]) {
      const int r = kk % st, jj = kk / st;
      const int Jr = (k - r + st - 1) / st;
      long base = 0;
      for (int q = 0; q < r; ++q) base += (long)Cin * ((k - q + st - 1) / st) * Cout;
      st_elem(d.Wb[l], base + (long)ci * (Jr * Cout) + (long)(Jr - 1 - jj) * Cout + co, d.dtype, v);
    }
  }
}
__global__ __launch_bounds__(256) void conv_wgrad_scatter_kernel(wavlm_conv_relayout_desc d, int accumulate) {
  const int l = blockIdx.y;
  const int Cout = d.Cout[l], Cin = d.Cin[l], k = d.k[l];
  const long n = (long)Cout * Cin * k;
  for (long e = (long)blockIdx.x * 256 + threadIdx.x; e < n; e += (long)gridDim.x * 256) {
    const int kk = (int)(e % k);
    const long t = e / k;
    const int ci = (int)(t % Cin), co = (int)(t / Cin);
    float v = ld_elem(d.Wf[l], (long)co * (k * Cin) + (long)kk * Cin + ci, d.dtype);
    if (accumulate) v += ld_elem(d.W[l], e, d.dtype);
    st_elem(const_cast<void*>(d.W[l]), e, d.dtype, v);
  }
}

extern "C" {

int wavlm_abi_version(void) { return WAVLM_HIP_ABI_VERSION; }
static double g_ln_prof_bytes = 0.0;
static bool ln_full_enabled() { static const bool on = !(getenv("WAVLM_LN_FULL") && getenv("WAVLM_LN_FULL")[0] == '0'); return on; }

int wavlm_layernorm_fwd(const void* x, const void* r, void* y, void* s, float* mean, float* rstd, const void* gamma,
                        const void* beta, int64_t rows, int32_t D, float eps, int32_t dtype, int32_t param_dtype,
                        int32_t act, float p_in, uint64_t seed_in, float p_out, uint64_t seed_out, void* stream) {
  if (!x || !y || !gamma || !beta || rows < 0 || D <= 0 || (D & 7) || D > LN_MAXC * 512) return WL_EINVAL;
  if (rows == 0) return WL_OK;
  hipStream_t st = (hipStream_t)stream;
  const unsigned ti = drop_thresh16(p_in), to = drop_thresh16(p_out);
  const float si = drop_scale16(ti), so = drop_scale16(to);
  {
    const double es = dtype == WL_BF16 ? 2.0 : 4.0;
    g_ln_prof_bytes = (double)rows * D * es * (2.0 + (r ? 1.0 : 0.0) + (s ? 1.0 : 0.0));
  }
  WlProfScope prof(WL_PROF_LN_FWD, dtype, 8.0 * rows * D, g_ln_prof_bytes, st);
  const unsigned grid = grid_for(rows, 4, (ti | to) ? LN_FWD_DROP_BLOCKS : 8192);
  if (ln_full_enabled() && (D == 512 || D == 768 || D == 1024) && (mean == nullptr) == (rstd == nullptr) && (!s || mean)) {
    static const int cap_env = getenv("WAVLM_LN_FWD_BLOCKS") ? atoi(getenv("WAVLM_LN_FWD_BLOCKS")) : 0;
    long cap = cap_env > 0 ? cap_env : rows / 128;
    if (cap_env <= 0) { if (cap < 1024) cap = 1024; if (cap > 8192) cap = 8192; }
    const unsigned gridf = grid_for(rows, 4, (unsigned)cap);
    static const bool gt_on = !(getenv("WAVLM_LN_GELU_TAB") && getenv("WAVLM_LN_GELU_TAB")[0] == '0');
    if (gt_on && act == 1 && dtype == WL_BF16 && param_dtype == WL_BF16 && D == 512 && !r && !(ti | to)) {
      const float4* gtab = wl_gelu_tab4(st);
      if (!gtab) return WL_ELAUNCH;
      if (mean)
        WL_LAUNCH((layernorm_fwd_full_kernel<bf16_t, bf16_t, 8, 1, false, true, true>), dim3(gridf), dim3(256), 0, st, (const bf16_t*)x,
                  (const bf16_t*)r, (bf16_t*)y, (bf16_t*)s, mean, rstd, (const bf16_t*)gamma, (const bf16_t*)beta, (long)rows, eps, (int)act,
                  ti, si, (unsigned long long)seed_in, to, so, (unsigned long long)seed_out, gtab);
      else
        WL_LAUNCH((layernorm_fwd_full_kernel<bf16_t, bf16_t, 8, 1, false, false, true>), dim3(gridf), dim3(256), 0, st, (const bf16_t*)x,
                  (const bf16_t*)r, (bf16_t*)y, (bf16_t*)s, mean, rstd, (const bf16_t*)gamma, (const bf16_t*)beta, (long)rows, eps, (int)act,
                  ti, si, (unsigned long long)seed_in, to, so, (unsigned long long)seed_out, gtab);
      return wl_check_launch();
    }
#define LNF_K(T, TP, VEC, NCS, HR, HS) WL_LAUNCH((layernorm_fwd_full_kernel<T, TP, VEC, NCS, HR, HS>), dim3(gridf), dim3(256), 0, st, \
    (const T*)x, (const T*)r, (T*)y, (T*)s, mean, rstd, (const TP*)gamma, (const TP*)beta, (long)rows, eps, (int)act, ti, si, \
    (unsigned long long)seed_in, to, so, (unsigned long long)seed_out)
#define LNF_W(T, TP, HR, HS) do { if (D == 512) LNF_K(T, TP, 8, 1, HR, HS); else if (D == 768) LNF_K(T, TP, 4, 3, HR, HS); else LNF_K(T, TP, 8, 2, HR, HS); } while (0)
#define LNF(T, TP) do { if (r) { if (mean) LNF_W(T, TP, true, true); else LNF_W(T, TP, true, false); } \
                        else { if (mean) LNF_W(T, TP, false, true); else LNF_W(T, TP, false, false); } } while (0)
    if (dtype == WL_F32 && param_dtype == WL_F32) LNF(float, float);
    else if (dtype == WL_BF16 && param_dtype == WL_BF16) LNF(bf16_t, bf16_t);
    else if (dtype == WL_BF16 && param_dtype == WL_F32) LNF(bf16_t, float);
    else return WL_EINVAL;
#undef LNF
#undef LNF_W
#undef LNF_K
    return wl_check_launch();
  }
#define LN_FWD_N(T, TP, NCS) WL_LAUNCH((layernorm_fwd_kernel<T, TP, NCS>), dim3(grid), dim3(256), 0, st, (const T*)x, \
    (const T*)r, (T*)y, (T*)s, mean, rstd, (const TP*)gamma, (const TP*)beta, (long)rows, (int)D, eps, (int)act, ti, si, \
    (unsigned long long)seed_in, to, so, (unsigned long long)seed_out)
#define LN_FWD(T, TP) do { if (D <= 512) LN_FWD_N(T, TP, 1); else if (D <= 1024) LN_FWD_N(T, TP, 2); else LN_FWD_N(T, TP, 4); } while (0)
  if (dtype == WL_F32 && param_dtype == WL_F32) LN_FWD(float, float);
  else if (dtype == WL_BF16 && param_dtype == WL_BF16) LN_FWD(bf16_t, bf16_t);
  else if (dtype == WL_BF16 && param_dtype == WL_F32) LN_FWD(bf16_t, float);
  else return WL_EINVAL;
#undef LN_FWD
#undef LN_FWD_N
  return wl_check_launch();
}

#define LN_BWD_BLOCKS_MAX 4096
static int ln_bwd_blocks_env() { static const int n = getenv("WAVLM_LN_BWD_BLOCKS") ? atoi(getenv("WAVLM_LN_BWD_BLOCKS")) : 0; return n > 0 && n <= LN_BWD_BLOCKS_MAX ? n : 0; }
static int ln_bwd_blocks(long rows) {
  if (ln_bwd_blocks_env()) return ln_bwd_blocks_env();
// ... 90 lines not shown
                     (int)param_dtype, (int)accumulate_params, (long)D, dbeta, dr_colsum);
  rc = wl_check_launch();
  if (rc == WL_OK && accumulate_params) {
    const uint64_t nb = (uint64_t)D * wl_esize(param_dtype);
    wl_notify_grad(dgamma, nb, stream); wl_notify_grad(dbeta, nb, stream);
    if (dr_colsum) wl_notify_grad(dr_colsum, nb, stream);
  }
  return rc;
}

}
int wl_colsum_finish(const float* part, int nblk, int n, void* out, int out_dtype, int accumulate, hipStream_t st) {
  if (wl_fin_add(part, nblk, (long)n, n, out, out_dtype, accumulate)) return WL_OK;
  WL_LAUNCH(colsum_finish_kernel, dim3((unsigned)((n + 15) / 16)), dim3(1024), 0, st, part, nblk, (long)n, n, out, out_dtype,
            accumulate, 0L, (void*)nullptr, (void*)nullptr);
  return wl_check_launch();
}
extern "C" {

uint64_t wavlm_colsum_workspace_bytes(int32_t N) { return (uint64_t)CS_BLOCKS * N * sizeof(float); }

int wavlm_colsum(const void* x, int64_t rows, int32_t N, int64_t ld, int32_t dtype, const uint8_t* include_mask,
                 const uint8_t* exclude_mask, void* out, int32_t out_dtype, int32_t accumulate, void* workspace,
                 uint64_t ws_bytes, void* stream) {
  if (!x || !out || !workspace || rows < 0 || N <= 0 || (N & 7) || N > CS_MAXC * 512 || (ld & 7)) return WL_EINVAL;
  if (ws_bytes < wavlm_colsum_workspace_bytes(N)) return WL_EINVAL;
  hipStream_t st = (hipStream_t)stream;
  const unsigned grid = grid_for(rows > 0 ? rows : 1, 4, CS_BLOCKS);
  float* part = (float*)workspace;
  if (dtype == WL_F32)
    WL_LAUNCH((colsum_partial_kernel<float>), dim3(grid), dim3(256), 0, st, (const float*)x, (long)rows, (int)N,
                       (long)ld, include_mask, exclude_mask, part);
  else if (dtype == WL_BF16)
    WL_LAUNCH((colsum_partial_kernel<bf16_t>), dim3(grid), dim3(256), 0, st, (const bf16_t*)x, (long)rows, (int)N,
                       (long)ld, include_mask, exclude_mask, part);
  else return WL_EINVAL;
  int rc = wl_check_launch();
  if (rc != WL_OK) return rc;
  if (wl_fin_add(part, (int)grid, (long)N, N, out, out_dtype, accumulate)) return WL_OK;
  WL_LAUNCH(colsum_finish_kernel, dim3((unsigned)((N + 15) / 16)), dim3(1024), 0, st, part, (int)grid, (long)N,
                     (int)N, out, (int)out_dtype, (int)accumulate, 0L, (void*)nullptr, (void*)nullptr);
  rc = wl_check_launch();
  if (rc == WL_OK && accumulate) wl_notify_grad(out, (uint64_t)N * wl_esize(out_dtype), stream);
  return rc;
}

int wavlm_select_rows(const void* x, void* y, const uint8_t* sel, const void* emb, const uint8_t* zero, int64_t rows,
                      int32_t D, int32_t dtype, int32_t emb_dtype, void* stream) {
  if (!x || !y || rows < 0 || D <= 0 || (D & 7)) return WL_EINVAL;
  if (rows == 0) return WL_OK;
  hipStream_t st = (hipStream_t)stream;
  const unsigned grid = grid_for(rows * (D >> 3), 256, 4096);
#define SEL(T, TP) WL_LAUNCH((select_rows_kernel<T, TP>), dim3(grid), dim3(256), 0, st, (const T*)x, (T*)y, sel, \
    (const TP*)emb, zero, (long)rows, (int)D)
  if (dtype == WL_F32 && emb_dtype == WL_F32) SEL(float, float);
  else if (dtype == WL_BF16 && emb_dtype == WL_BF16) SEL(bf16_t, bf16_t);
  else if (dtype == WL_BF16 && emb_dtype == WL_F32) SEL(bf16_t, float);
  else return WL_EINVAL;
#undef SEL
  return wl_check_launch();
}

int wavlm_gather_rows(const void* src, const int32_t* idx, void* dst, int64_t n_out, int32_t D, int32_t dtype,
                      void* stream) {
  if (!src || !idx || !dst || n_out < 0 || D <= 0 || (D & 7)) return WL_EINVAL;
  if (n_out == 0) return WL_OK;
  hipStream_t st = (hipStream_t)stream;
  const unsigned grid = grid_for(n_out * (D >> 3), 256, 4096);
  if (dtype == WL_F32)
    WL_LAUNCH((gather_rows_kernel<float>), dim3(grid), dim3(256), 0, st, (const float*)src, idx, (float*)dst,
                       (long)n_out, (int)D);
  else if (dtype == WL_BF16)
    WL_LAUNCH((gather_rows_kernel<bf16_t>), dim3(grid), dim3(256), 0, st, (const bf16_t*)src, idx, (bf16_t*)dst,
                       (long)n_out, (int)D);
  else return WL_EINVAL;
  return wl_check_launch();
}

int wavlm_conv_weights_relayout(const wavlm_conv_relayout_desc* d, void* stream) {
  if (!d || d->n_layers < 1 || d->n_layers > WL_CONV_RELAYOUT_MAX || (d->dtype != WL_F32 && d->dtype != WL_BF16)) return WL_EINVAL;
  long mx = 0;
  for (int l = 0; l < d->n_layers; ++l) {
    if (!d->W[l] || !d->Wf[l] || d->Cout[l] <= 0 || d->Cin[l] <= 0 || d->k[l] <= 0 || d->s[l] <= 0 || d->s[l] > d->k[l]) return WL_EINVAL;
    const long n = (long)d->Cout[l] * d->Cin[l] * d->k[l];
    if (n > mx) mx = n;
  }
  const unsigned gx = grid_for(mx, 256, 8192);
  WL_LAUNCH(conv_weights_relayout_kernel, dim3(gx, (unsigned)d->n_layers), dim3(256), 0, (hipStream_t)stream, *d);
  return wl_check_launch();
}

int wavlm_conv_wgrad_scatter(const wavlm_conv_relayout_desc* d, int32_t accumulate, void* stream) {
  if (!d || d->n_layers < 1 || d->n_layers > WL_CONV_RELAYOUT_MAX || (d->dtype != WL_F32 && d->dtype != WL_BF16)) return WL_EINVAL;
  long mx = 0;
  for (int l = 0; l < d->n_layers; ++l) {
    if (!d->W[l] || !d->Wf[l] || d->Cout[l] <= 0 || d->Cin[l] <= 0 || d->k[l] <= 0) return WL_EINVAL;
    const long n = (long)d->Cout[l] * d->Cin[l] * d->k[l];
    if (n > mx) mx = n;
  }
  const unsigned gx = grid_for(mx, 256, 8192);
  WL_LAUNCH(conv_wgrad_scatter_kernel, dim3(gx, (unsigned)d->n_layers), dim3(256), 0, (hipStream_t)stream, *d, (int)accumulate);
  const int rc = wl_check_launch();
  if (rc == WL_OK && accumulate)
    for (int l = 0; l < d->n_layers; ++l)
      wl_notify_grad(d->W[l], (uint64_t)d->Cout[l] * d->Cin[l] * d->k[l] * wl_esize(d->dtype), stream);
  return rc;
}

int wavlm_axpby(const void* x, int32_t x_dtype, void* y, int32_t y_dtype, int64_t n, float a, float b, void* stream) {
  if (!x || !y || n < 0) return WL_EINVAL;
  if (n == 0) return WL_OK;
  WL_LAUNCH(axpby_kernel, dim3(grid_for(n, 256, 8192)), dim3(256), 0, (hipStream_t)stream, x, (int)x_dtype, y,
                     (int)y_dtype, (long)n, a, b);
  return wl_check_launch();
}

int wavlm_scale_dev(void* y, int32_t dtype, int64_t n, const float* scalar, float extra, void* stream) {
  if (!y || !scalar || n < 0) return WL_EINVAL;
  if (n == 0) return WL_OK;
  WL_LAUNCH(scale_dev_kernel, dim3(grid_for(n, 256, 8192)), dim3(256), 0, (hipStream_t)stream, y, (int)dtype,
                     (long)n, scalar, extra);
  return wl_check_launch();
}

int wavlm_dropout(const void* x, void* y, int64_t n, float p, uint64_t seed, int32_t dtype, void* stream) {
  if (!x || !y || n < 0 || (n & 7) || p < 0.f || p >= 1.f) return WL_EINVAL;
  if (n == 0) return WL_OK;
  hipStream_t st = (hipStream_t)stream;
  const unsigned th = drop_thresh(p);
  const float sc = 1.f / (1.f - p);
  const unsigned grid = grid_for(n >> 3, 256, 8192);
  if (dtype == WL_F32)
    WL_LAUNCH((dropout_kernel<float>), dim3(grid), dim3(256), 0, st, (const float*)x, (float*)y, (long)(n >> 3), th,
                       sc, (unsigned long long)seed);
  else if (dtype == WL_BF16)
    WL_LAUNCH((dropout_kernel<bf16_t>), dim3(grid), dim3(256), 0, st, (const bf16_t*)x, (bf16_t*)y,
                       (long)(n >> 3), th, sc, (unsigned long long)seed);
  else return WL_EINVAL;
  return wl_check_launch();
}

int wavlm_dropout_add(const void* x, const void* r, void* y, int64_t n, float p, uint64_t seed, int32_t dtype, void* stream) {
  if (!x || !r || !y || n < 0 || (n & 7) || p < 0.f || p >= 1.f) return WL_EINVAL;
  if (n == 0) return WL_OK;
  hipStream_t st = (hipStream_t)stream;
  const unsigned th = p > 0.f ? drop_thresh(p) : 0u;
  const float sc = 1.f / (1.f - p);
  const unsigned grid = grid_for(n >> 3, 256, 8192);
  if (dtype == WL_F32)
    WL_LAUNCH((dropout_add_kernel<float>), dim3(grid), dim3(256), 0, st, (const float*)x, (const float*)r, (float*)y,
              (long)(n >> 3), th, sc, (unsigned long long)seed);
  else if (dtype == WL_BF16)
    WL_LAUNCH((dropout_add_kernel<bf16_t>), dim3(grid), dim3(256), 0, st, (const bf16_t*)x, (const bf16_t*)r, (bf16_t*)y,
              (long)(n >> 3), th, sc, (unsigned long long)seed);
  else return WL_EINVAL;
  return wl_check_launch();
}

int wavlm_replace_mix(const void* x, const void* q, const uint8_t* sel, void* y, int64_t rows, int32_t D, float p, uint64_t seed,
                      int32_t dtype, void* stream) {
  if (!x || !q || !sel || !y || rows < 0 || D <= 0 || (D & 7) || p < 0.f || p >= 1.f) return WL_EINVAL;
  if (dtype != WL_F32 && dtype != WL_BF16) return WL_EINVAL;
  if (rows == 0) return WL_OK;
  hipStream_t st = (hipStream_t)stream;
  const unsigned th = drop_thresh(p);
  const float sc = 1.f / (1.f - p);
  const long n8 = (long)rows * (D >> 3);
  const unsigned grid = grid_for(n8, 256, 8192);
  if (dtype == WL_F32)
    WL_LAUNCH((replace_mix_kernel<float>), dim3(grid), dim3(256), 0, st, (const float*)x, (const float*)q, sel, (float*)y, n8,
              (int)(D >> 3), th, sc, (unsigned long long)seed);
  else
    WL_LAUNCH((replace_mix_kernel<bf16_t>), dim3(grid), dim3(256), 0, st, (const bf16_t*)x, (const bf16_t*)q, sel, (bf16_t*)y,
              n8, (int)(D >> 3), th, sc, (unsigned long long)seed);
  return wl_check_launch();
}

int wavlm_replace_mix_bwd(const void* g, const uint8_t* sel, void* dx, void* dq, int64_t rows, int32_t D, float p, uint64_t seed,
                          int32_t dtype, void* stream) {
  if (!g || !sel || !dx || !dq || rows < 0 || D <= 0 || (D & 7) || p < 0.f || p >= 1.f) return WL_EINVAL;
  if (dtype != WL_F32 && dtype != WL_BF16) return WL_EINVAL;
  if (rows == 0) return WL_OK;
  hipStream_t st = (hipStream_t)stream;
// ... 30 lines not shown
```

Measured before the change: 14790 audio-s/s.

## Defer split-K and dtab reductions into merged finish kernel; tile conv weight relayouts

Split-K grouped GEMM reductions and the attention relative-position-bias gradient reduction can now be queued into the deferred finish list and run inside one merged colsum finish launch instead of separate kernels. The weight-grad path keeps its workspace slabs alive while merging, so the deferred reductions still see valid partial sums. Separately, the conv weight relayout and wgrad scatter kernels gain a shared-memory tiled path that uses vectorized 8-wide loads and stores instead of per-element strided access. The aim is fewer kernel launches and better memory coalescing, at the cost of more workspace held live and a larger, more branchy finish kernel.

```diff
diff --git a/unispeech_amd/csrc/attn_fused.hip b/unispeech_amd/csrc/attn_fused.hip
--- a/unispeech_amd/csrc/attn_fused.hip
+++ b/unispeech_amd/csrc/attn_fused.hip
@@ -1,4 +1,5 @@
 #include "attn_fused.hpp"
+#include "fin_segments.hpp"
 
 typedef float f32x2_t __attribute__((ext_vector_type(2)));
 #if !defined(WAVLM_EXPERIMENTAL)
@@ -818,55 +819,9 @@
   }
 }
 
-__global__ __launch_bounds__(1024) void fa_dtab_reduce_kernel(const float* __restrict__ part, float* __restrict__ out,
-                                                              int B, int H, int nqt, int L, int Lp, int T, int nkv, int accumulate) {
+__global__ __launch_bounds__(1024) void fa_dtab_reduce_kernel(WlFinDtab p) {
   __shared__ float4 red[64][17];
-  const int col = threadIdx.x & 15, slice = threadIdx.x >> 4;
-  const int d = (blockIdx.x * 16 + col) * 4;
-  const int h = blockIdx.y;
-  const int nrow = nqt * 4, ntot = B * nrow, span = 64 * nkv + 32;
-  float4 acc[4];
-#pragma unroll
-  for (int u = 0; u < 4; ++u) acc[u] = make_float4(0.f, 0.f, 0.f, 0.f);
-  if (d < Lp) {
-    for (int r0 = slice; r0 < ntot; r0 += 256) {
-#pragma unroll
-      for (int u = 0; u < 4; ++u) {
-        const int r = r0 + 64 * u;
-        if (r < ntot) {
-          const int b = r / nrow, c = r - b * nrow;
-          const int k0 = d - (T - 1 - 32 * c - 31);
-          if (k0 > -4 && k0 < span) {
-            const float4 v = *reinterpret_cast<const float4*>(part + (((long)b * H + h) * nrow + c) * Lp + d);
-            acc[u].x += (k0 >= 0 && k0 < span) ? v.x : 0.f;
-            acc[u].y += (k0 + 1 >= 0 && k0 + 1 < span) ? v.y : 0.f;
-            acc[u].z += (k0 + 2 >= 0 && k0 + 2 < span) ? v.z : 0.f;
-            acc[u].w += (k0 + 3 >= 0 && k0 + 3 < span) ? v.w : 0.f;
-          }
-        }
-      }
-    }
-  }
-  float4 t;
-  t.x = (acc[0].x + acc[1].x) + (acc[2].x + acc[3].x); t.y = (acc[0].y + acc[1].y) + (acc[2].y + acc[3].y);
-  t.z = (acc[0].z + acc[1].z) + (acc[2].z + acc[3].z); t.w = (acc[0].w + acc[1].w) + (acc[2].w + acc[3].w);
-  red[slice][col] = t;
-  __syncthreads();
-  if (slice < 4) {
-    float4 q = make_float4(0.f, 0.f, 0.f, 0.f);
-#pragma unroll
-    for (int k = 0; k < 16; ++k) { const float4 v = red[slice * 16 + k][col]; q.x += v.x; q.y += v.y; q.z += v.z; q.w += v.w; }
-    red[slice * 16][col] = q;
-  }
-  __syncthreads();
-  if (slice == 0 && d < L) {
-    const float4 a0 = red[0][col], a1 = red[16][col], a2 = red[32][col], a3 = red[48][col];
-    const float o[4] = {(a0.x + a1.x) + (a2.x + a3.x), (a0.y + a1.y) + (a2.y + a3.y), (a0.z + a1.z) + (a2.z + a3.z),
-                        (a0.w + a1.w) + (a2.w + a3.w)};
-#pragma unroll
-    for (int k = 0; k < 4; ++k)
-      if (d + k < L) out[(long)h * L + d + k] = accumulate ? out[(long)h * L + d + k] + o[k] : o[k];
-  }
+  wl_dtab_reduce_body(p, (int)blockIdx.x, (int)blockIdx.y, red);
 }
 
 static FaP fa_params(int B, int H, int T, float scale, float p_drop, uint64_t seed) {
@@ -1055,8 +1010,12 @@
     if (rcb != WL_OK) return rcb;
     if (dbias_accumulate && !wl_fin_active()) wl_notify_grad(dbias, (uint64_t)3 * H * FA_HD * wl_esize(dbias_dtype), stream);
   }
-  if (tab)
-    WL_LAUNCH(fa_dtab_reduce_kernel, dim3((unsigned)((Lp / 4 + 15) / 16), (unsigned)H), dim3(1024), 0, st,
-              (const float*)p.dtab_part, dtab, (int)B, (int)H, nqt, L, Lp, (int)T, (T + FA_BKV - 1) / FA_BKV, (int)dtab_accumulate);
+  if (tab) {
+    WlFinDtab r;
+    r.part = p.dtab_part; r.out = dtab; r.B = B; r.H = H; r.nqt = nqt; r.L = L; r.Lp = Lp; r.T = T;
+    r.nkv = (T + FA_BKV - 1) / FA_BKV; r.accumulate = dtab_accumulate; r.nbx = (Lp / 4 + 15) / 16;
+    if (!wl_fin_add_dtab(r))
+      WL_LAUNCH(fa_dtab_reduce_kernel, dim3((unsigned)r.nbx, (unsigned)H), dim3(1024), 0, st, r);
+  }
   return wl_check_launch();
 }
diff --git a/unispeech_amd/csrc/common.hpp b/unispeech_amd/csrc/common.hpp
--- a/unispeech_amd/csrc/common.hpp
+++ b/unispeech_amd/csrc/common.hpp
@@ -195,10 +195,22 @@
 int wl_colsum_finish(const float* part, int nblk, int n, void* out, int out_dtype, int accumulate, hipStream_t st);
 
 struct WlFinSeg { const float* part; void* out; long stride, rep_stride; int nblk, n, out_dtype, accumulate, rep, blk0; };
+struct WlFinDtab { const float* part; float* out; int B, H, nqt, L, Lp, T, nkv, accumulate, nbx; };
+struct WlFinRed {
+  float* ws[4]; void* C[4]; long ldc[4]; int M[4], N[4], c_dtype[4], accumulate[4]; float alpha[4];
+  long base[5]; int n, S, nblk;
+};
 #define WL_FIN_MAX 16
-struct WlFinList { WlFinSeg s[WL_FIN_MAX]; int n, blocks; };
+#define WL_FIN_MAX_RED 2
+struct WlFinList {
+  WlFinSeg s[WL_FIN_MAX]; WlFinDtab dtab; WlFinRed red[WL_FIN_MAX_RED];
+  int n, blocks, ndtab, nred, red_blk0[WL_FIN_MAX_RED], dtab_blk0, cs_blk0;
+};
 void wl_fin_defer(WlFinList* l);
 bool wl_fin_active();
+bool wl_fin_merging();
 bool wl_fin_add(const float* part, int nblk, long stride, int n, void* out, int out_dtype, int accumulate, int rep = 1,
                 long rep_stride = 0);
+bool wl_fin_add_dtab(const WlFinDtab& d);
+bool wl_fin_add_red(const WlFinRed& r);
 int wl_fin_flush(WlFinList& l, void* stream);
diff --git a/unispeech_amd/csrc/fin_segments.hpp b/unispeech_amd/csrc/fin_segments.hpp
--- /dev/null
+++ b/unispeech_amd/csrc/fin_segments.hpp
@@ -0,0 +1,145 @@
+#pragma once
+#include "common.hpp"
+
+__device__ __forceinline__ void ld8_dt(const void* p, long idx, int dt, float (&v)[8]) {
+  if (dt == WL_F32) {
+    const float4 a = *reinterpret_cast<const float4*>((const float*)p + idx);
+    const float4 b = *reinterpret_cast<const float4*>((const float*)p + idx + 4);
+    v[0] = a.x; v[1] = a.y; v[2] = a.z; v[3] = a.w; v[4] = b.x; v[5] = b.y; v[6] = b.z; v[7] = b.w;
+  } else {
+    const uint4 a = *reinterpret_cast<const uint4*>((const bf16_t*)p + idx);
+    v[0] = __uint_as_float(a.x << 16); v[1] = __uint_as_float(a.x & 0xffff0000u);
+    v[2] = __uint_as_float(a.y << 16); v[3] = __uint_as_float(a.y & 0xffff0000u);
+    v[4] = __uint_as_float(a.z << 16); v[5] = __uint_as_float(a.z & 0xffff0000u);
+    v[6] = __uint_as_float(a.w << 16); v[7] = __uint_as_float(a.w & 0xffff0000u);
+  }
+}
+__device__ __forceinline__ void st8_dt(void* p, long idx, int dt, const float (&v)[8]) {
+  if (dt == WL_F32) {
+    *reinterpret_cast<float4*>((float*)p + idx) = make_float4(v[0], v[1], v[2], v[3]);
+    *reinterpret_cast<float4*>((float*)p + idx + 4) = make_float4(v[4], v[5], v[6], v[7]);
+  } else {
+    uint4 o;
+    o.x = pack_bf16x2(v[0], v[1]); o.y = pack_bf16x2(v[2], v[3]);
+    o.z = pack_bf16x2(v[4], v[5]); o.w = pack_bf16x2(v[6], v[7]);
+    *reinterpret_cast<uint4*>((bf16_t*)p + idx) = o;
+  }
+}
+
+__device__ __forceinline__ void wl_red_grouped_body(const WlFinRed& p, long first, long step) {
+  const long total8 = p.base[p.n];
+  for (long i8 = first; i8 < total8; i8 += step) {
+    const int g = (i8 >= p.base[1]) + (i8 >= p.base[2]) + (i8 >= p.base[3]);
+    const long i = (i8 - p.base[g]) << 3;
+    const int N = p.N[g];
+    const long mn = (long)p.M[g] * N;
+    const float* src = p.ws[g] + i;
+    float v[8];
+#pragma unroll
+    for (int e = 0; e < 8; ++e) v[e] = 0.f;
+    for (int k = 0; k < p.S; ++k) {
+      const float4 a = *reinterpret_cast<const float4*>(src + (long)k * mn);
+      const float4 b = *reinterpret_cast<const float4*>(src + (long)k * mn + 4);
+      v[0] += a.x; v[1] += a.y; v[2] += a.z; v[3] += a.w; v[4] += b.x; v[5] += b.y; v[6] += b.z; v[7] += b.w;
+    }
+    const long m = i / N, n = i - m * N;
+    const long off = m * p.ldc[g] + n;
+#pragma unroll
+    for (int e = 0; e < 8; ++e) v[e] *= p.alpha[g];
+    if (p.accumulate[g]) {
+      float c[8];
+      ld8_dt(p.C[g], off, p.c_dtype[g], c);
+#pragma unroll
+      for (int e = 0; e < 8; ++e) v[e] += c[e];
+    }
+    st8_dt(p.C[g], off, p.c_dtype[g], v);
+  }
+}
+
+__device__ __forceinline__ void wl_dtab_reduce_body(const WlFinDtab& p, int bx, int h, float4 (*red)[17]) {
+  const float* __restrict__ part = p.part;
+  float* __restrict__ out = p.out;
+  const int H = p.H, L = p.L, Lp = p.Lp, T = p.T;
+  const int col = threadIdx.x & 15, slice = threadIdx.x >> 4;
+  const int d = (bx * 16 + col) * 4;
+  const int nrow = p.nqt * 4, ntot = p.B * nrow, span = 64 * p.nkv + 32;
+  float4 acc[4];
+#pragma unroll
+  for (int u = 0; u < 4; ++u) acc[u] = make_float4(0.f, 0.f, 0.f, 0.f);
+  if (d < Lp) {
+    for (int r0 = slice; r0 < ntot; r0 += 256) {
+#pragma unroll
+      for (int u = 0; u < 4; ++u) {
+        const int r = r0 + 64 * u;
+        if (r < ntot) {
+          const int b = r / nrow, c = r - b * nrow;
+          const int k0 = d - (T - 1 - 32 * c - 31);
+          if (k0 > -4 && k0 < span) {
+            const float4 v = *reinterpret_cast<const float4*>(part + (((long)b * H + h) * nrow + c) * Lp + d);
+            acc[u].x += (k0 >= 0 && k0 < span) ? v.x : 0.f;
+            acc[u].y += (k0 + 1 >= 0 && k0 + 1 < span) ? v.y : 0.f;
+            acc[u].z += (k0 + 2 >= 0 && k0 + 2 < span) ? v.z : 0.f;
+            acc[u].w += (k0 + 3 >= 0 && k0 + 3 < span) ? v.w : 0.f;
+          }
+        }
+      }
+    }
+  }
+  float4 t;
+  t.x = (acc[0].x + acc[1].x) + (acc[2].x + acc[3].x); t.y = (acc[0].y + acc[1].y) + (acc[2].y + acc[3].y);
+  t.z = (acc[0].z + acc[1].z) + (acc[2].z + acc[3].z); t.w = (acc[0].w + acc[1].w) + (acc[2].w + acc[3].w);
+  red[slice][col] = t;
+  __syncthreads();
+  if (slice < 4) {
+    float4 q = make_float4(0.f, 0.f, 0.f, 0.f);
+#pragma unroll
+    for (int k = 0; k < 16; ++k) { const float4 v = red[slice * 16 + k][col]; q.x += v.x; q.y += v.y; q.z += v.z; q.w += v.w; }
+    red[slice * 16][col] = q;
+  }
+  __syncthreads();
+  if (slice == 0 && d < L) {
+    const float4 a0 = red[0][col], a1 = red[16][col], a2 = red[32][col], a3 = red[48][col];
+    const float o[4] = {(a0.x + a1.x) + (a2.x + a3.x), (a0.y + a1.y) + (a2.y + a3.y), (a0.z + a1.z) + (a2.z + a3.z),
+                        (a0.w + a1.w) + (a2.w + a3.w)};
+#pragma unroll
+    for (int k = 0; k < 4; ++k)
+      if (d + k < L) out[(long)h * L + d + k] = p.accumulate ? out[(long)h * L + d + k] + o[k] : o[k];
+  }
+}
+
+__device__ __forceinline__ void wl_colsum_seg_body(const WlFinSeg& g, int bx, float (*red)[17]) {
+  const float* __restrict__ part = g.part;
+  const long stride = g.stride;
+  const int nblk = g.nblk, n = g.n;
+  const int col = threadIdx.x & 15, slice = threadIdx.x >> 4;
+  const int c = bx * 16 + col;
+  float s = 0.f;
+  if (c < n) {
+    float s0 = 0.f, s1 = 0.f, s2 = 0.f, s3 = 0.f;
+    int b = slice;
+    for (; b + 192 < nblk; b += 256) {
+      s0 += part[(long)b * stride + c];
+      s1 += part[(long)(b + 64) * stride + c];
+      s2 += part[(long)(b + 128) * stride + c];
+      s3 += part[(long)(b + 192) * stride + c];
+    }
+    for (; b < nblk; b += 64) s0 += part[(long)b * stride + c];
+    s = (s0 + s1) + (s2 + s3);
+  }
+  red[slice][col] = s;
+  __syncthreads();
+  if (slice < 4) {
+    float t = 0.f;
+#pragma unroll
+    for (int k = 0; k < 16; ++k) t += red[slice * 16 + k][col];
+    red[slice * 16][col] = t;
+  }
+  __syncthreads();
+  if (slice == 0 && c < n) {
+    s = (red[0][col] + red[16][col]) + (red[32][col] + red[48][col]);
+    for (int r = 0; r < g.rep; ++r) {
+      const long idx = (long)r * g.rep_stride + c;
+      st_elem(g.out, idx, g.out_dtype, g.accumulate ? s + ld_elem(g.out, idx, g.out_dtype) : s);
+    }
+  }
+}
diff --git a/unispeech_amd/csrc/gemm_bf16.hip b/unispeech_amd/csrc/gemm_bf16.hip
--- a/unispeech_amd/csrc/gemm_bf16.hip
+++ b/unispeech_amd/csrc/gemm_bf16.hip
@@ -189,38 +189,8 @@
   }
 }
 
-struct RedGrpP {
-  float* ws[4]; void* C[4]; long ldc[4]; int M[4], N[4], c_dtype[4], accumulate[4]; float alpha[4];
-  long base[5]; int n, S;
-};
-__global__ __launch_bounds__(256) void gemm_splitk_reduce8_grouped_kernel(RedGrpP p) {
-  const long total8 = p.base[p.n];
-  for (long i8 = (long)blockIdx.x * blockDim.x + threadIdx.x; i8 < total8; i8 += (long)gridDim.x * blockDim.x) {
-    const int g = (i8 >= p.base[1]) + (i8 >= p.base[2]) + (i8 >= p.base[3]);
-    const long i = (i8 - p.base[g]) << 3;
-    const int N = p.N[g];
-    const long mn = (long)p.M[g] * N;
-    const float* src = p.ws[g] + i;
-    float v[8];
-#pragma unroll
-    for (int e = 0; e < 8; ++e) v[e] = 0.f;
-    for (int k = 0; k < p.S; ++k) {
-      const float4 a = *reinterpret_cast<const float4*>(src + (long)k * mn);
-      const float4 b = *reinterpret_cast<const float4*>(src + (long)k * mn + 4);
-      v[0] += a.x; v[1] += a.y; v[2] += a.z; v[3] += a.w; v[4] += b.x; v[5] += b.y; v[6] += b.z; v[7] += b.w;
-    }
-    const long m = i / N, n = i - m * N;
-    const long off = m * p.ldc[g] + n;
-#pragma unroll
-    for (int e = 0; e < 8; ++e) v[e] *= p.alpha[g];
-    if (p.accumulate[g]) {
-      float c[8];
-      ld8_dt(p.C[g], off, p.c_dtype[g], c);
-#pragma unroll
-      for (int e = 0; e < 8; ++e) v[e] += c[e];
-    }
-    st8_dt(p.C[g], off, p.c_dtype[g], v);
-  }
+__global__ __launch_bounds__(256) void gemm_splitk_reduce8_grouped_kernel(WlFinRed p) {
+  wl_red_grouped_body(p, (long)blockIdx.x * blockDim.x + threadIdx.x, (long)gridDim.x * blockDim.x);
 }
 
 template <bool TA, bool TB, int BM, int BN, int WM, int WN>
@@ -606,9 +576,10 @@
   const bool fixup = w4_takes(d, true) && gemm_w4_fixup_ok(p);
   p.fix_epoch = fixup ? 1u : 0u; p.fix_cnt = nullptr; p.fix_flag = nullptr;
   int rc = w4_takes(d, true) ? gemm_w4_launch_grouped(p, st) : gemm_pp_launch_grouped(p, st);
+  bool deferred = false;
   if (rc == WL_OK && !fixup) {
-    RedGrpP r;
-    r.n = n; r.S = p.split_k; r.base[0] = 0;
+    WlFinRed r;
+    r.n = n; r.S = p.split_k; r.nblk = 0; r.base[0] = 0;
     for (int i = 0; i < 4; ++i) {
       const wavlm_gemm_desc* e = d + (i < n ? i : n - 1);
       r.ws[i] = (float*)e->workspace; r.C[i] = e->C; r.ldc[i] = e->ldc; r.M[i] = e->M; r.N[i] = e->N;
@@ -616,12 +587,15 @@
       r.base[i + 1] = i < n ? r.base[i] + (((long)e->M * e->N) >> 3) : 0x7fffffffffffffffL;
     }
     const long total8 = r.base[n];
-    long blocks = (total8 + 255) / 256; if (blocks > 4096) blocks = 4096;
-    WL_LAUNCH(gemm_splitk_reduce8_grouped_kernel, dim3((unsigned)blocks), dim3(256), 0, st, r);
-    rc = wl_check_launch();
+    deferred = wl_fin_add_red(r);
+    if (!deferred) {
+      long blocks = (total8 + 255) / 256; if (blocks > 4096) blocks = 4096;
+      WL_LAUNCH(gemm_splitk_reduce8_grouped_kernel, dim3((unsigned)blocks), dim3(256), 0, st, r);
+      rc = wl_check_launch();
+    }
   }
   prof_end(pi, st);
-  if (rc == WL_OK)
+  if (rc == WL_OK && !deferred)
     for (int i = 0; i < n; ++i) gemm_notify(d + i, false, stream);
   return rc;
 }
diff --git a/unispeech_amd/csrc/gemm_common.hpp b/unispeech_amd/csrc/gemm_common.hpp
--- a/unispeech_amd/csrc/gemm_common.hpp
+++ b/unispeech_amd/csrc/gemm_common.hpp
@@ -1,6 +1,7 @@
 #pragma once
 #include <stdlib.h>
 #include "common.hpp"
+#include "fin_segments.hpp"
 #include "../../include/wavlm_hip.h"
 
 struct GemmGrp { const void* A; const void* B; float* ws; long lda, ldb; int M, N, tiles_m, tiles_n, vbase;
@@ -127,30 +128,6 @@
 }
 
 
-__device__ __forceinline__ void ld8_dt(const void* p, long idx, int dt, float (&v)[8]) {
-  if (dt == WL_F32) {
-    const float4 a = *reinterpret_cast<const float4*>((const float*)p + idx);
-    const float4 b = *reinterpret_cast<const float4*>((const float*)p + idx + 4);
-    v[0] = a.x; v[1] = a.y; v[2] = a.z; v[3] = a.w; v[4] = b.x; v[5] = b.y; v[6] = b.z; v[7] = b.w;
-  } else {
-    const uint4 a = *reinterpret_cast<const uint4*>((const bf16_t*)p + idx);
-    v[0] = __uint_as_float(a.x << 16); v[1] = __uint_as_float(a.x & 0xffff0000u);
-    v[2] = __uint_as_float(a.y << 16); v[3] = __uint_as_float(a.y & 0xffff0000u);
-    v[4] = __uint_as_float(a.z << 16); v[5] = __uint_as_float(a.z & 0xffff0000u);
-    v[6] = __uint_as_float(a.w << 16); v[7] = __uint_as_float(a.w & 0xffff0000u);
-  }
-}
-__device__ __forceinline__ void st8_dt(void* p, long idx, int dt, const float (&v)[8]) {
-  if (dt == WL_F32) {
-    *reinterpret_cast<float4*>((float*)p + idx) = make_float4(v[0], v[1], v[2], v[3]);
-    *reinterpret_cast<float4*>((float*)p + idx + 4) = make_float4(v[4], v[5], v[6], v[7]);
-  } else {
-    uint4 o;
-    o.x = pack_bf16x2(v[0], v[1]); o.y = pack_bf16x2(v[2], v[3]);
-    o.z = pack_bf16x2(v[4], v[5]); o.w = pack_bf16x2(v[6], v[7]);
-    *reinterpret_cast<uint4*>((bf16_t*)p + idx) = o;
-  }
-}
 
 __device__ __forceinline__ void gemm_store8(const GemmP& p, int zo, int zi, int z, int split, int m, int n,
                                             float (&acc)[8]) {
diff --git a/unispeech_amd/csrc/layer.hip b/unispeech_amd/csrc/layer.hip
--- a/unispeech_amd/csrc/layer.hip
+++ b/unispeech_amd/csrc/layer.hip
@@ -197,8 +197,11 @@
   for (int i = 0; i < cnt; ++i)
     if (!it[i].dy || !it[i].x || !it[i].dW || it[i].N <= 0 || it[i].K <= 0) return WL_EINVAL;
   const long kt = (long)((n + 63) / 64);
+  const bool keep_slabs = wl_fin_merging();
+  Carver c(ws, wsb);
   int i = 0;
   while (i < cnt) {
+    if (!keep_slabs) c.off = 0;
     int j = i; long tiles = 0;
     while (wl_policy::grouping() && j < cnt && j - i < 4) {
       const long t = wg_tiles(it[j]);
@@ -207,7 +210,6 @@
     }
     if (j == i) j = i + 1;
     const int m = j - i;
-    Carver c(ws, wsb);
     if (m >= 2) {
       const int split = wavlm_slabs_grouped(tiles, kt, 0, -1, -1);
       wavlm_gemm_desc g[4];
diff --git a/unispeech_amd/csrc/posconv.hip b/unispeech_amd/csrc/posconv.hip
--- a/unispeech_amd/csrc/posconv.hip
+++ b/unispeech_amd/csrc/posconv.hip
@@ -1,4 +1,5 @@
 #include "common.hpp"
+#include "fin_segments.hpp"
 #include "../../include/wavlm_hip.h"
 
 #define PC_BLOCKS 512
@@ -37,8 +38,67 @@
   }
 }
 
+__device__ __forceinline__ void pc_ld8(const float* p, float (&v)[8]) { ld8_dt(p, 0, WL_F32, v); }
+__device__ __forceinline__ void pc_ld8(const bf16_t* p, float (&v)[8]) { ld8_dt(p, 0, WL_BF16, v); }
+__device__ __forceinline__ void pc_st8(float* p, const float (&v)[8]) { st8_dt(p, 0, WL_F32, v); }
+__device__ __forceinline__ void pc_st8(bf16_t* p, const float (&v)[8]) { st8_dt(p, 0, WL_BF16, v); }
+
 template <typename TP, typename TO>
 __global__ __launch_bounds__(256) void pc_weight_kernel(const TP* __restrict__ v, const TP* __restrict__ g,
+    const float* __restrict__ norm, TO* __restrict__ Wf, TO* __restrict__ Wb, int D, int Cg, int K, int layout) {
+  extern __shared__ float pc_wt[];
+  const int KP = K + 1;
+  float* gk = pc_wt + 64 * KP;
+  float* nk = gk + K;
+  for (int k = threadIdx.x; k < K; k += 256) { gk[k] = Elem<TP>::ld(g + k); nk[k] = norm[k]; }
+  __syncthreads();
+  const long KC = (long)K * Cg;
+  const int ct = Cg >> 3;
+  const int cit = blockIdx.x % ct, cot = (blockIdx.x / ct) % ct, grp = blockIdx.x / (ct * ct);
+  auto off = [&](int n, int tap, int c) -> long {
+    if (layout == 0) return ((long)grp * Cg + n) * KC + (long)tap * Cg + c;
+    const int J = K >> 4;
+    return (long)grp * Cg * KC + (((((long)(c >> 3) * 4 + ((tap & 15) >> 2)) * J + (tap >> 4)) * 4 + (tap & 3)) * Cg + n) * 8 + (c & 7);
+  };
+  for (int q0 = threadIdx.x; q0 < 8 * K; q0 += 1024) {
+    float x[4][8];
+#pragma unroll
+    for (int u = 0; u < 4; ++u) {
+      const int q = q0 + 256 * u;
+      if (q < 8 * K) {
+        const int c = q / K, j = q - c * K;
+        pc_ld8(v + (((long)grp * Cg + cot * 8 + c) * Cg + cit * 8) * K + 8 * j, x[u]);
+      }
+    }
+#pragma unroll
+    for (int u = 0; u < 4; ++u) {
+      const int q = q0 + 256 * u;
+      if (q < 8 * K) {
+        const int c = q / K, j = q - c * K;
+        int ci = 8 * j / K, k = 8 * j - ci * K;
+#pragma unroll
+        for (int e = 0; e < 8; ++e) {
+          pc_wt[(c * 8 + ci) * KP + k] = gk[k] * x[u][e] / nk[k];
+          if (++k == K) { k = 0; ++ci; }
+        }
+      }
+    }
+  }
+  __syncthreads();
+  for (int q = threadIdx.x; q < 8 * K; q += 256) {
+    const int c = layout == 0 ? q / K : q & 7, k = layout == 0 ? q - c * K : q >> 3;
+    float w[8];
+#pragma unroll
+    for (int e = 0; e < 8; ++e) w[e] = pc_wt[(c * 8 + e) * KP + k];
+    pc_st8(Wf + off(cot * 8 + c, k, cit * 8), w);
+#pragma unroll
+    for (int e = 0; e < 8; ++e) w[e] = pc_wt[(e * 8 + c) * KP + k];
+    pc_st8(Wb + off(cit * 8 + c, K - 1 - k, cot * 8), w);
+  }
+}
+
+template <typename TP, typename TO>
+__global__ __launch_bounds__(256) void pc_weight_elem_kernel(const TP* __restrict__ v, const TP* __restrict__ g,
     const float* __restrict__ norm, TO* __restrict__ Wf, TO* __restrict__ Wb, int D, int Cg, int K, int layout) {
   const long total = (long)D * Cg * K;
   const long KC = (long)K * Cg;
@@ -59,23 +119,50 @@
   }
 }
 
+template <bool VEC>
 __global__ __launch_bounds__(256) void pc_unpack_dw_kernel(const float* __restrict__ dWf, float* __restrict__ dw, int D,
                                                            int Cg, int K, int nsplit) {
   extern __shared__ float pc_tile[];
   const int co = blockIdx.x;
   const long n = (long)K * Cg, total = (long)D * n;
   const float* src = dWf + (long)co * n;
-  for (int i = threadIdx.x; i < (int)n; i += 256) {
-    float a = src[i];
-    for (int sidx = 1; sidx < nsplit; ++sidx) a += src[sidx * total + i];
-    const int k = i / Cg, ci = i - k * Cg;
-    pc_tile[k * (Cg + 1) + ci] = a;
-  }
-  __syncthreads();
   float* dst = dw + (long)co * n;
-  for (int i = threadIdx.x; i < (int)n; i += 256) {
-    const int ci = i / K, k = i - ci * K;
-    dst[i] = pc_tile[k * (Cg + 1) + ci];
+  if constexpr (VEC) {
+    for (int i = 4 * threadIdx.x; i < (int)n; i += 1024) {
+      float4 a = *reinterpret_cast<const float4*>(src + i);
+      for (int sidx = 1; sidx < nsplit; ++sidx) {
+        const float4 b = *reinterpret_cast<const float4*>(src + sidx * total + i);
+        a.x += b.x; a.y += b.y; a.z += b.z; a.w += b.w;
+      }
+      const float e[4] = {a.x, a.y, a.z, a.w};
+#pragma unroll
+      for (int u = 0; u < 4; ++u) {
+        const int k = (i + u) / Cg, ci = (i + u) - k * Cg;
+        pc_tile[k * (Cg + 1) + ci] = e[u];
+      }
+    }
+    __syncthreads();
+    for (int i = 4 * threadIdx.x; i < (int)n; i += 1024) {
+      float e[4];
+#pragma unroll
+      for (int u = 0; u < 4; ++u) {
+        const int ci = (i + u) / K, k = (i + u) - ci * K;
+        e[u] = pc_tile[k * (Cg + 1) + ci];
+      }
+      *reinterpret_cast<float4*>(dst + i) = make_float4(e[0], e[1], e[2], e[3]);
+    }
+  } else {
+    for (int i = threadIdx.x; i < (int)n; i += 256) {
+      float a = src[i];
+      for (int sidx = 1; sidx < nsplit; ++sidx) a += src[sidx * total + i];
+      const int k = i / Cg, ci = i - k * Cg;
+      pc_tile[k * (Cg + 1) + ci] = a;
+    }
+    __syncthreads();
+    for (int i = threadIdx.x; i < (int)n; i += 256) {
+      const int ci = i / K, k = i - ci * K;
+      dst[i] = pc_tile[k * (Cg + 1) + ci];
+    }
   }
 }
 template <typename TP>
@@ -151,23 +238,29 @@
   const unsigned th = (unsigned)((K + 63) / 64 * 64);
   const long total = rows * K;
   long grid = (total + 255) / 256; if (grid > 4096) grid = 4096;
+  const size_t smem = ((size_t)64 * (K + 1) + 2 * (size_t)K) * sizeof(float);
+  const bool tiled = (Cg & 7) == 0 && smem <= 65536 && (((uintptr_t)v | (uintptr_t)Wf | (uintptr_t)Wb) & 15) == 0;
+  const unsigned tgrid = (unsigned)((D / Cg) * (Cg >> 3) * (Cg >> 3));
+#define PC_WEIGHT(TP, TO)                                                                                              \
+  do {                                                                                                                 \
+    if (tiled) WL_LAUNCH((pc_weight_kernel<TP, TO>), dim3(tgrid), dim3(256), smem, st, (const TP*)v, (const TP*)g, norm, \
+                         (TO*)Wf, (TO*)Wb, (int)D, (int)Cg, (int)K, (int)layout);                                      \
+    else WL_LAUNCH((pc_weight_elem_kernel<TP, TO>), dim3((unsigned)grid), dim3(256), 0, st, (const TP*)v, (const TP*)g,  \
+                   norm, (TO*)Wf, (TO*)Wb, (int)D, (int)Cg, (int)K, (int)layout);                                      \
+  } while (0)
   if (param_dtype == WL_F32) {
     WL_LAUNCH((pc_rowdot_partial_kernel<float, float>), dim3(PC_BLOCKS), dim3(th), 0, st, (const float*)v,
                        (const float*)v, rows, (int)K, part);
     WL_LAUNCH(pc_finish_kernel, dim3((unsigned)((K + 15) / 16)), dim3(1024), 0, st, part, PC_BLOCKS, (int)K, norm, 1);
-    if (out_dtype == WL_F32)
-      WL_LAUNCH((pc_weight_kernel<float, float>), dim3((unsigned)grid), dim3(256), 0, st, (const float*)v,
-                         (const float*)g, norm, (float*)Wf, (float*)Wb, (int)D, (int)Cg, (int)K, (int)layout);
-    else
-      WL_LAUNCH((pc_weight_kernel<float, bf16_t>), dim3((unsigned)grid), dim3(256), 0, st, (const float*)v,
-                         (const float*)g, norm, (bf16_t*)Wf, (bf16_t*)Wb, (int)D, (int)Cg, (int)K, (int)layout);
+    if (out_dtype == WL_F32) PC_WEIGHT(float, float);
+    else PC_WEIGHT(float, bf16_t);
   } else if (param_dtype == WL_BF16 && out_dtype == WL_BF16) {
     WL_LAUNCH((pc_rowdot_partial_kernel<bf16_t, bf16_t>), dim3(PC_BLOCKS), dim3(th), 0, st, (const bf16_t*)v,
                        (const bf16_t*)v, rows, (int)K, part);
     WL_LAUNCH(pc_finish_kernel, dim3((unsigned)((K + 15) / 16)), dim3(1024), 0, st, part, PC_BLOCKS, (int)K, norm, 1);
-    WL_LAUNCH((pc_weight_kernel<bf16_t, bf16_t>), dim3((unsigned)grid), dim3(256), 0, st, (const bf16_t*)v,
-                       (const bf16_t*)g, norm, (bf16_t*)Wf, (bf16_t*)Wb, (int)D, (int)Cg, (int)K, (int)layout);
+    PC_WEIGHT(bf16_t, bf16_t);
   } else return WL_EINVAL;
+#undef PC_WEIGHT
   return wl_check_launch();
 }
 
@@ -186,7 +279,11 @@
   const long total = rows * K;
   long grid = (total + 255) / 256; if (grid > 4096) grid = 4096;
   const unsigned th = (unsigned)((K + 63) / 64 * 64);
-  WL_LAUNCH(pc_unpack_dw_kernel, dim3((unsigned)D), dim3(256), (size_t)K * (Cg + 1) * sizeof(float), st, dWf, dw, (int)D, (int)Cg, (int)K, (int)nsplit);
+  const size_t tile_b = (size_t)K * (Cg + 1) * sizeof(float);
+  if (((long)K * Cg) % 4 == 0 && (((uintptr_t)dWf | (uintptr_t)dw) & 15) == 0)
+    WL_LAUNCH(pc_unpack_dw_kernel<true>, dim3((unsigned)D), dim3(256), tile_b, st, dWf, dw, (int)D, (int)Cg, (int)K, (int)nsplit);
+  else
+    WL_LAUNCH(pc_unpack_dw_kernel<false>, dim3((unsigned)D), dim3(256), tile_b, st, dWf, dw, (int)D, (int)Cg, (int)K, (int)nsplit);
   if (param_dtype == WL_F32) {
     WL_LAUNCH((pc_rowdot_partial_kernel<float, float>), dim3(PC_BLOCKS), dim3(th), 0, st, (const float*)dw,
                        (const float*)v, rows, (int)K, part);
diff --git a/unispeech_amd/csrc/rowops.hip b/unispeech_amd/csrc/rowops.hip
--- a/unispeech_amd/csrc/rowops.hip
+++ b/unispeech_amd/csrc/rowops.hip
@@ -1,4 +1,5 @@
 #include "common.hpp"
+#include "fin_segments.hpp"
 #include <stdlib.h>
 #include "../../include/wavlm_hip.h"
 
@@ -557,50 +558,31 @@
 }
 
 __global__ __launch_bounds__(1024) void colsum_finish_multi_kernel(WlFinList L) {
-  __shared__ float red[64][17];
+  __shared__ float4 red4[64][17];
+  const int bid = (int)blockIdx.x;
+  if (bid < L.dtab_blk0) {
+    const int k = (L.nred > 1 && bid >= L.red_blk0[1]) ? 1 : 0;
+    const WlFinRed& r = L.red[k];
+    wl_red_grouped_body(r, (long)(bid - L.red_blk0[k]) * 1024 + threadIdx.x, (long)r.nblk * 1024);
+    return;
+  }
+  if (bid < L.cs_blk0) {
+    const int b = bid - L.dtab_blk0;
+    wl_dtab_reduce_body(L.dtab, b % L.dtab.nbx, b / L.dtab.nbx, red4);
+    return;
+  }
+  const int cb = bid - L.cs_blk0;
   int si = 0;
 #pragma unroll 1
-  for (int k = 1; k < L.n; ++k) if ((int)blockIdx.x >= L.s[k].blk0) si = k;
-  const WlFinSeg& g = L.s[si];
-  const float* __restrict__ part = g.part;
-  const long stride = g.stride;
-  const int nblk = g.nblk, n = g.n;
-  const int col = threadIdx.x & 15, slice = threadIdx.x >> 4;
-  const int c = ((int)blockIdx.x - g.blk0) * 16 + col;
-  float s = 0.f;
-  if (c < n) {
-    float s0 = 0.f, s1 = 0.f, s2 = 0.f, s3 = 0.f;
-    int b = slice;
-    for (; b + 192 < nblk; b += 256) {
-      s0 += part[(long)b * stride + c];
-      s1 += part[(long)(b + 64) * stride + c];
-      s2 += part[(long)(b + 128) * stride + c];
-      s3 += part[(long)(b + 192) * stride + c];
-    }
-    for (; b < nblk; b += 64) s0 += part[(long)b * stride + c];
-    s = (s0 + s1) + (s2 + s3);
-  }
-  red[slice][col] = s;
-  __syncthreads();
-  if (slice < 4) {
-    float t = 0.f;
-#pragma unroll
-    for (int k = 0; k < 16; ++k) t += red[slice * 16 + k][col];
-    red[slice * 16][col] = t;
-  }
-  __syncthreads();
-  if (slice == 0 && c < n) {
-    s = (red[0][col] + red[16][col]) + (red[32][col] + red[48][col]);
-    for (int r = 0; r < g.rep; ++r) {
-      const long idx = (long)r * g.rep_stride + c;
-      st_elem(g.out, idx, g.out_dtype, g.accumulate ? s + ld_elem(g.out, idx, g.out_dtype) : s);
-    }
-  }
+  for (int k = 1; k < L.n; ++k) if (cb >= L.s[k].blk0) si = k;
+  wl_colsum_seg_body(L.s[si], cb - L.s[si].blk0, reinterpret_cast<float (*)[17]>(red4));
 }
 
 static thread_local WlFinList* g_fin_list = nullptr;
-void wl_fin_defer(WlFinList* l) { g_fin_list = l; if (l) { l->n = 0; l->blocks = 0; } }
+static bool fin_merge_enabled() { static const bool on = !(getenv("WAVLM_FIN_MERGE") && getenv("WAVLM_FIN_MERGE")[0] == '0'); return on; }
+void wl_fin_defer(WlFinList* l) { g_fin_list = l; if (l) { l->n = 0; l->blocks = 0; l->ndtab = 0; l->nred = 0; } }
 bool wl_fin_active() { return g_fin_list != nullptr; }
+bool wl_fin_merging() { return g_fin_list != nullptr && fin_merge_enabled(); }
 bool wl_fin_add(const float* part, int nblk, long stride, int n, void* out, int out_dtype, int accumulate, int rep, long rep_stride) {
   WlFinList* l = g_fin_list;
   if (!l || l->n >= WL_FIN_MAX || n <= 0) return false;
@@ -610,16 +592,44 @@
   l->blocks += (n + 15) / 16;
   return true;
 }
+bool wl_fin_add_dtab(const WlFinDtab& d) {
+  WlFinList* l = g_fin_list;
+  if (!l || !fin_merge_enabled() || l->ndtab || d.nbx <= 0 || d.H <= 0) return false;
+  l->dtab = d; l->ndtab = 1;
+  return true;
+}
+bool wl_fin_add_red(const WlFinRed& r) {
+  WlFinList* l = g_fin_list;
+  if (!l || !fin_merge_enabled() || l->nred >= WL_FIN_MAX_RED || r.n < 1 || r.n > 4 || r.base[r.n] <= 0) return false;
+  WlFinRed& q = l->red[l->nred++];
+  q = r;
+  long nb = (r.base[r.n] + 1023) / 1024; if (nb > 1024) nb = 1024;
+  q.nblk = (int)nb;
+  return true;
+}
 int wl_fin_flush(WlFinList& l, void* stream) {
-  if (l.n == 0) return WL_OK;
-  WL_LAUNCH(colsum_finish_multi_kernel, dim3((unsigned)l.blocks), dim3(1024), 0, (hipStream_t)stream, l);
+  if (l.n == 0 && l.ndtab == 0 && l.nred == 0) return WL_OK;
+  int blk = 0;
+  l.red_blk0[0] = l.red_blk0[1] = 0;
+  for (int k = 0; k < l.nred; ++k) { l.red_blk0[k] = blk; blk += l.red[k].nblk; }
+  l.dtab_blk0 = blk;
+  if (l.ndtab) blk += l.dtab.nbx * l.dtab.H;
+  l.cs_blk0 = blk;
+  blk += l.blocks;
+  WL_LAUNCH(colsum_finish_multi_kernel, dim3((unsigned)blk), dim3(1024), 0, (hipStream_t)stream, l);
   const int rc = wl_check_launch();
-  if (rc == WL_OK)
+  if (rc == WL_OK) {
     for (int k = 0; k < l.n; ++k) {
       const WlFinSeg& g = l.s[k];
       if (g.accumulate) wl_notify_grad(g.out, (uint64_t)((long)(g.rep - 1) * g.rep_stride + g.n) * wl_esize(g.out_dtype), stream);
     }
-  l.n = 0; l.blocks = 0;
+    for (int k = 0; k < l.nred; ++k) {
+      const WlFinRed& r = l.red[k];
+      for (int g = 0; g < r.n; ++g)
+        if (r.accumulate[g]) wl_notify_grad(r.C[g], ((uint64_t)(r.M[g] - 1) * r.ldc[g] + r.N[g]) * wl_esize(r.c_dtype[g]), stream);
+    }
+  }
+  l.n = 0; l.blocks = 0; l.ndtab = 0; l.nred = 0;
   return rc;
 }
 
@@ -840,8 +850,66 @@
 #endif
 #define CS_BLOCKS 512
 
+#define CR_MAXK 16
+#define CR_CI 64
+struct ConvTile { int Cout, Cin, k, st, co0, ci0, nci; };
+__host__ __device__ __forceinline__ bool conv_relayout_tiled(const wavlm_conv_relayout_desc& d, int l, bool need_wb) {
+  const uintptr_t a = (uintptr_t)d.W[l] | (uintptr_t)d.Wf[l] | (need_wb ? (uintptr_t)d.Wb[l] : 0);
+  return (d.Cin[l] & 7) == 0 && (d.Cout[l] & 7) == 0 && d.k[l] <= CR_MAXK && (a & 15) == 0;
+}
+__host__ __device__ __forceinline__ long conv_ntiles(const wavlm_conv_relayout_desc& d, int l) {
+  return (long)((d.Cin[l] + CR_CI - 1) / CR_CI) * (d.Cout[l] >> 3);
+}
+__device__ __forceinline__ ConvTile conv_tile_at(const wavlm_conv_relayout_desc& d, int l, long b) {
+  ConvTile t;
+  t.Cout = d.Cout[l]; t.Cin = d.Cin[l]; t.k = d.k[l]; t.st = d.s[l];
+  const int cit = (t.Cin + CR_CI - 1) / CR_CI;
+  t.co0 = (int)(b / cit) * 8; t.ci0 = (int)(b % cit) * CR_CI;
+  t.nci = t.Cin - t.ci0 < CR_CI ? t.Cin - t.ci0 : CR_CI;
+  return t;
+}
+__device__ __forceinline__ long conv_wb_off(const ConvTile& t, int ci, int co, int kk) {
+  const int r = kk % t.st, jj = kk / t.st;
+  const int Jr = (t.k - r + t.st - 1) / t.st;
+  long base = 0;
+  for (int q = 0; q < r; ++q) base += (long)t.Cin * ((t.k - q + t.st - 1) / t.st) * t.Cout;
+  return base + (long)ci * (Jr * t.Cout) + (long)(Jr - 1 - jj) * t.Cout + co;
+}
 __global__ __launch_bounds__(256) void conv_weights_relayout_kernel(wavlm_conv_relayout_desc d) {
+  __shared__ float tile[8 * (CR_CI * CR_MAXK + 1)];
   const int l = blockIdx.y;
+  if (conv_relayout_tiled(d, l, d.Wb[l] != nullptr)) {
+    for (long b = blockIdx.x; b < conv_ntiles(d, l); b += gridDim.x) {
+      const ConvTile t = conv_tile_at(d, l, b);
+      const int run = t.nci * t.k, rp = CR_CI * CR_MAXK + 1, nv = run >> 3;
+      for (int q = threadIdx.x; q < 8 * nv; q += 256) {
+        const int c = q / nv, j = q - c * nv;
+        float x[8];
+        ld8_dt(d.W[l], ((long)(t.co0 + c) * t.Cin + t.ci0) * t.k + 8 * j, d.dtype, x);
+#pragma unroll
+        for (int e = 0; e < 8; ++e) tile[c * rp + 8 * j + e] = x[e];
+      }
+      __syncthreads();
+      const int c8n = t.nci >> 3;
+      for (int q = threadIdx.x; q < 8 * t.k * c8n; q += 256) {
+        const int c8 = q % c8n, kk = (q / c8n) % t.k, c = q / (c8n * t.k);
+        float x[8];
+#pragma unroll
+        for (int e = 0; e < 8; ++e) x[e] = tile[c * rp + (c8 * 8 + e) * t.k + kk];
+        st8_dt(d.Wf[l], (long)(t.co0 + c) * (t.k * t.Cin) + (long)kk * t.Cin + t.ci0 + c8 * 8, d.dtype, x);
+      }
+      if (d.Wb[l])
+        for (int q = threadIdx.x; q < t.nci * t.k; q += 256) {
+          const int kk = q % t.k, ci = q / t.k;
+          float x[8];
+#pragma unroll
+          for (int e = 0; e < 8; ++e) x[e] = tile[e * rp + ci * t.k + kk];
+          st8_dt(d.Wb[l], conv_wb_off(t, t.ci0 + ci, t.co0, kk), d.dtype, x);
+        }
+      __syncthreads();
+    }
+    return;
+  }
   const int Cout = d.Cout[l], Cin = d.Cin[l], k = d.k[l], st = d.s[l];
   const long n = (long)Cout * Cin * k;
   for (long e = (long)blockIdx.x * 256 + threadIdx.x; e < n; e += (long)gridDim.x * 256) {
@@ -860,7 +928,38 @@
   }
 }
 __global__ __launch_bounds__(256) void conv_wgrad_scatter_kernel(wavlm_conv_relayout_desc d, int accumulate) {
+  __shared__ float tile[8 * (CR_CI * CR_MAXK + 1)];
   const int l = blockIdx.y;
+  if (conv_relayout_tiled(d, l, false)) {
+    for (long b = blockIdx.x; b < conv_ntiles(d, l); b += gridDim.x) {
+      const ConvTile t = conv_tile_at(d, l, b);
+      const int run = t.nci * t.k, rp = CR_CI * CR_MAXK + 1, nv = run >> 3, c8n = t.nci >> 3;
+      for (int q = threadIdx.x; q < 8 * t.k * c8n; q += 256) {
+        const int c8 = q % c8n, kk = (q / c8n) % t.k, c = q / (c8n * t.k);
+        float x[8];
+        ld8_dt(d.Wf[l], (long)(t.co0 + c) * (t.k * t.Cin) + (long)kk * t.Cin + t.ci0 + c8 * 8, d.dtype, x);
+#pragma unroll
+        for (int e = 0; e < 8; ++e) tile[c * rp + (c8 * 8 + e) * t.k + kk] = x[e];
+      }
+      __syncthreads();
+      for (int q = threadIdx.x; q < 8 * nv; q += 256) {
+        const int c = q / nv, j = q - c * nv;
+        const long o = ((long)(t.co0 + c) * t.Cin + t.ci0) * t.k + 8 * j;
+        float x[8];
+#pragma unroll
+        for (int e = 0; e < 8; ++e) x[e] = tile[c * rp + 8 * j + e];
+        if (accumulate) {
+          float g[8];
+          ld8_dt(d.W[l], o, d.dtype, g);
+#pragma unroll
+          for (int e = 0; e < 8; ++e) x[e] += g[e];
+        }
+        st8_dt(const_cast<void*>(d.W[l]), o, d.dtype, x);
+      }
+      __syncthreads();
+    }
+    return;
+  }
   const int Cout = d.Cout[l], Cin = d.Cin[l], k = d.k[l];
   const long n = (long)Cout * Cin * k;
   for (long e = (long)blockIdx.x * 256 + threadIdx.x; e < n; e += (long)gridDim.x * 256) {
@@ -1117,10 +1216,10 @@
   long mx = 0;
   for (int l = 0; l < d->n_layers; ++l) {
     if (!d->W[l] || !d->Wf[l] || d->Cout[l] <= 0 || d->Cin[l] <= 0 || d->k[l] <= 0 || d->s[l] <= 0 || d->s[l] > d->k[l]) return WL_EINVAL;
-    const long n = (long)d->Cout[l] * d->Cin[l] * d->k[l];
+    const long n = conv_relayout_tiled(*d, l, d->Wb[l] != nullptr) ? conv_ntiles(*d, l) : ((long)d->Cout[l] * d->Cin[l] * d->k[l] + 255) / 256;
     if (n > mx) mx = n;
   }
-  const unsigned gx = grid_for(mx, 256, 8192);
+  const unsigned gx = grid_for(mx, 1, 8192);
   WL_LAUNCH(conv_weights_relayout_kernel, dim3(gx, (unsigned)d->n_layers), dim3(256), 0, (hipStream_t)stream, *d);
   return wl_check_launch();
 }
@@ -1130,10 +1229,10 @@
   long mx = 0;
   for (int l = 0; l < d->n_layers; ++l) {
     if (!d->W[l] || !d->Wf[l] || d->Cout[l] <= 0 || d->Cin[l] <= 0 || d->k[l] <= 0) return WL_EINVAL;
-    const long n = (long)d->Cout[l] * d->Cin[l] * d->k[l];
+    const long n = conv_relayout_tiled(*d, l, false) ? conv_ntiles(*d, l) : ((long)d->Cout[l] * d->Cin[l] * d->k[l] + 255) / 256;
     if (n > mx) mx = n;
   }
-  const unsigned gx = grid_for(mx, 256, 8192);
+  const unsigned gx = grid_for(mx, 1, 8192);
   WL_LAUNCH(conv_wgrad_scatter_kernel, dim3(gx, (unsigned)d->n_layers), dim3(256), 0, (hipStream_t)stream, *d, (int)accumulate);
   const int rc = wl_check_launch();
   if (rc == WL_OK && accumulate)
```

After: 14890 audio-s/s, median of 6. Within noise of the previous version (+0.7%).
